# brendisurfs/Distributed-Backtesting-Exploration

Hardware: AMD Instinct MI355X
Metric: bar-evals/sec (symbols x params x bars) (higher is better)
Workload: dtype f64+int64; 1 GPU; BASELINE config 2: SMA fast/slow crossover, 5,000 symbols x 2,520 daily bars x 400 params per GPU; symbols_total=5000, symbols_per_gpu=5000, bars=2520, params=400, topk=100, parallelism=dp1 (contiguous symbol shards; exchange: none)

## Files before the change

distributed-backtesting-exploration_amd/csrc/analysis.cpp:

```cpp
#include <algorithm>
#include <cstring>
#include <string>
#include <vector>

#include "covariance.h"
#include "engine_state.h"
#include "portfolio.h"
#include "replay.h"
#include "surface.h"
#include "topk_rules.h"
#include "walkfwd.h"

using namespace bt;

namespace {

[[noreturn]] void refuse(const char* fn, const std::string& why) { throw HipFail{std::string(fn) + ": " + why}; }

uint8_t* enter(bt_engine* e, size_t staging_bytes) {
    activate(e);
    sync_all(e);
    e->d_arena.ensure(staging_bytes);
    return e->d_arena.p;
}

template <class F>
void for_chunks(size_t n, size_t per, F fn) {
    for (size_t i0 = 0; i0 < n; i0 += per) fn(i0, std::min(per, n - i0));
}

int32_t replay_impl(bt_engine* e, int32_t n, const bt_lane* lanes, int32_t trade_cap, bt_summary* sum,
                    int32_t* n_bars, bt_trade* trades, int64_t* equity, int8_t* pos, int64_t stride) {
    const char* fn = "bt_replay";
    if (!e) refuse(fn, "null engine");
    std::string why = replay_refusal(!e->syms.empty(), n, trade_cap, trades != nullptr, lanes != nullptr, sum != nullptr);
    if (!why.empty()) refuse(fn, why);
    if (n == 0) return 0;
    std::vector<ReplayLane> req;
    int32_t W = 0;
    why = replay_resolve(e->syms.data(), e->syms.size(), e->P, n, lanes, equity || pos, stride, req, W);
    if (!why.empty()) refuse(fn, why);
    const ReplayPlan pl = plan_replay(n, W, trade_cap, stride, equity != nullptr, pos != nullptr);
    uint8_t* base = enter(e, pl.staging_bytes);
    const size_t dcap = (size_t)pl.dcap, pitch = (size_t)pl.pitch;
    ReplayLane* d_lanes = at<ReplayLane>(base, pl.o_lane);
    ReplayOut out{};
    out.sum = at<bt_summary>(base, pl.o_sum);
    out.trades = dcap ? at<bt_trade>(base, pl.o_trades) : nullptr;
    out.trade_cap = (int32_t)dcap;
    out.equity = equity ? at<int64_t>(base, pl.o_equity) : nullptr;
    out.pos = pos ? at<int8_t>(base, pl.o_pos) : nullptr;
    out.pitch = pl.pitch;
    auto fetch = [&](void* dst, size_t dst_pitch, const void* src, size_t src_pitch, size_t m) {
        if (dst_pitch == src_pitch) {
            HIPCHK(hipMemcpyAsync(dst, src, m * src_pitch, hipMemcpyDeviceToHost, e->stream));
            return;
        }
        HIPCHK(hipMemcpy2DAsync(dst, dst_pitch, src, src_pitch, src_pitch, m, hipMemcpyDeviceToHost, e->stream));
        for (size_t i = 0; i < m; ++i)
            memset(static_cast<uint8_t*>(dst) + i * dst_pitch + src_pitch, 0, dst_pitch - src_pitch);
    };
    for_chunks((size_t)n, (size_t)pl.lanes_per_chunk, [&](size_t i0, size_t m) {
        HIPCHK(hipMemcpyAsync(d_lanes, req.data() + i0, m * sizeof(ReplayLane), hipMemcpyHostToDevice, e->stream));
        if (dcap) HIPCHK(hipMemsetAsync(out.trades, 0, m * dcap * sizeof(bt_trade), e->stream));
        if (equity) HIPCHK(hipMemsetAsync(out.equity, 0, m * pitch * 8, e->stream));
        if (pos) HIPCHK(hipMemsetAsync(out.pos, 0, m * pitch, e->stream));
        HIPCHK(launch_replay(d_lanes, (int32_t)m, e->d_h.p, e->d_l.p, e->d_c.p, e->grid, out, e->stream));
        HIPCHK(hipMemcpyAsync(sum + i0, out.sum, m * sizeof(bt_summary), hipMemcpyDeviceToHost, e->stream));
        if (dcap)
            fetch(trades + i0 * (size_t)trade_cap, (size_t)trade_cap * sizeof(bt_trade), out.trades,
                  dcap * sizeof(bt_trade), m);
        if (equity) fetch(equity + i0 * (size_t)stride, (size_t)stride * 8, out.equity, pitch * 8, m);
        if (pos) fetch(pos + i0 * (size_t)stride, (size_t)stride, out.pos, pitch, m);
        HIPCHK(hipStreamSynchronize(e->stream));
    });
    if (n_bars)
        for (int32_t i = 0; i < n; ++i) n_bars[i] = req[i].bars;
    return n;
}

void surface_launch(bt_engine* e, const SurfacePlan& pl, uint8_t* base, const bt_summary* d_sum,
                    const int32_t* d_ids, int32_t id_stride, int32_t S, int32_t P, bt_param_agg* agg,
                    bt_topk_rec* best) {
    SurfaceWork w{};
    w.partial = at<bt_param_agg>(base, pl.o_partial);
    w.fold = at<bt_param_agg>(base, pl.o_fold);
    w.best_partial = at<bt_topk_rec>(base, pl.o_best_partial);
    w.agg = agg ? at<bt_param_agg>(base, pl.o_agg) : nullptr;
    w.best = best ? at<bt_topk_rec>(base, pl.o_best) : nullptr;
    HIPCHK(launch_surface(d_sum, d_ids, id_stride, S, P, pl, w, e->stream));
    const size_t n_agg = (size_t)P * sizeof(bt_param_agg), n_best = (size_t)S * sizeof(bt_topk_rec);
    const size_t lo = agg ? pl.o_agg : pl.o_best, hi = best && S > 0 ? pl.o_best + n_best : pl.o_agg + n_agg;
    if (hi <= lo) return;
    e->h_surface.ensure(hi - lo);
    HIPCHK(hipMemcpyAsync(e->h_surface.p, base + lo, hi - lo, hipMemcpyDeviceToHost, e->stream));
    HIPCHK(hipStreamSynchronize(e->stream));
    if (agg) memcpy(agg, e->h_surface.p + (pl.o_agg - lo), n_agg);
    if (best && S > 0) memcpy(best, e->h_surface.p + (pl.o_best - lo), n_best);
}

int32_t surface_impl(bt_engine* e, bt_param_agg* agg, bt_topk_rec* best) {
    const char* fn = "bt_surface";
    if (!e) refuse(fn, "null engine");
    if (!e->ran) refuse(fn, "no results");
    uint64_t rows = 0;
    for (const SymDesc& sd : e->syms) rows += (uint64_t)sd.bars;
    const int32_t S = (int32_t)e->syms.size();
    const std::string why = surface_refusal(S, e->P, agg || best, false, rows);
    if (!why.empty()) refuse(fn, why);
    const SurfacePlan pl = plan_surface(S, e->P, e->cus, e->surface_chunks);
    uint8_t* base = enter(e, pl.staging_bytes);
    static_assert(sizeof(SymDesc) == 16 && offsetof(SymDesc, id) == 12, "SymDesc layout");
    surface_launch(e, pl, base, e->d_sum[e->cur].p, reinterpret_cast<const int32_t*>(e->d_syms.p) + 3, 4, S,
                   e->P, agg, best);
    return 0;
}

int32_t surface_of_impl(bt_engine* e, int32_t S, int32_t P, const bt_summary* sum, const int32_t* ids,
                        bt_param_agg* agg, bt_topk_rec* best) {
    const char* fn = "bt_surface_of";
    if (!e) refuse(fn, "null engine");
    const std::string why = surface_refusal(S, P, agg || best, true, 0);
    if (!why.empty()) refuse(fn, why);
    if (S > 0 && (!sum || !ids)) refuse(fn, "sum and sym_ids are required");
    const SurfacePlan pl = plan_surface(S, P, e->cus, e->surface_chunks, true);
    uint8_t* base = enter(e, pl.staging_bytes);
    bt_summary* d_sum = at<bt_summary>(base, pl.o_sum);
    int32_t* d_ids = at<int32_t>(base, pl.o_ids);
    if (S > 0) {
        HIPCHK(hipMemcpyAsync(d_sum, sum, (size_t)S * (size_t)P * sizeof(bt_summary), hipMemcpyHostToDevice, e->stream));
        HIPCHK(hipMemcpyAsync(d_ids, ids, (size_t)S * sizeof(int32_t), hipMemcpyHostToDevice, e->stream));
    }
    surface_launch(e, pl, base, d_sum, d_ids, 1, S, P, agg, best);
    return 0;
}

int32_t topk_of_impl(bt_engine* e, int32_t S, int32_t P, const bt_summary* sum, const int32_t* ids, int32_t k,
                     int32_t lds_free_hist, bt_topk_rec* out) {
    static_assert(kTopkOfMaxK == kTopkMax, "topk_rules.h restates kTopkMax");
    const char* fn = "bt_topk_of";
    if (!e) refuse(fn, "null engine");
    const std::string why = topk_of_refusal(S, P, k, sum != nullptr, ids, out != nullptr);
    if (!why.empty()) refuse(fn, why);
    const size_t n = (size_t)S * (size_t)P;
    std::vector<uint64_t> key(n);
    for (size_t i = 0; i < n; ++i) key[i] = order_key(sum[i].sharpe);
    std::vector<SymDesc> syms((size_t)S);
    for (int32_t s = 0; s < S; ++s) syms[s] = SymDesc{0, 0, ids[s]};
    const TopkOfPlan pl = plan_topk_of(S, P);
    uint8_t* base = enter(e, pl.staging_bytes);
    uint64_t* d_key = at<uint64_t>(base, pl.o_key);
    bt_summary* d_sum = at<bt_summary>(base, pl.o_sum);
    SymDesc* d_syms = at<SymDesc>(base, pl.o_syms);
    bt_topk_rec* d_out = at<bt_topk_rec>(base, pl.o_out);
    const TopkWork w{at<unsigned int>(base, pl.o_hist),      at<unsigned long long>(base, pl.o_state),
                     at<unsigned int>(base, pl.o_counts),    at<unsigned long long>(base, pl.o_above),
                     at<unsigned long long>(base, pl.o_cand), kTopkCap, d_out + 1, reinterpret_cast<int32_t*>(d_out)};
    HIPCHK(hipMemcpyAsync(d_key, key.data(), n * sizeof(uint64_t), hipMemcpyHostToDevice, e->stream));
    HIPCHK(hipMemcpyAsync(d_sum, sum, n * sizeof(bt_summary), hipMemcpyHostToDevice, e->stream));
    HIPCHK(hipMemcpyAsync(d_syms, syms.data(), (size_t)S * sizeof(SymDesc), hipMemcpyHostToDevice, e->stream));
    HIPCHK(hipMemsetAsync(d_out, 0, ((size_t)kTopkMax + 1) * sizeof(bt_topk_rec), e->stream));
    HIPCHK(launch_topk_init(w, e->stream));
    HIPCHK(launch_topk(d_key, d_sum, d_syms, (int64_t)n, P, k, w, e->stream, lds_free_hist != 0));
    std::vector<bt_topk_rec> got((size_t)k + 1);
    HIPCHK(hipMemcpyAsync(got.data(), d_out, got.size() * sizeof(bt_topk_rec), hipMemcpyDeviceToHost, e->stream));
    HIPCHK(hipStreamSynchronize(e->stream));
    int32_t count;
    memcpy(&count, &got[0], sizeof count);
    if (count < 0 || count > k) refuse(fn, "the device wrote a count of " + std::to_string(count));
    memcpy(out, got.data() + 1, (size_t)count * sizeof(bt_topk_rec));
    return count;
}

int32_t walk_forward_impl(bt_engine* e, int32_t K, const int32_t* bounds, int32_t train, bt_fold* folds,
                          bt_wf_step* steps, bt_fold* total) {
    const char* fn = "bt_walk_forward";
    if (!e) refuse(fn, "null engine");
    if (e->syms.empty()) refuse(fn, "no dataset loaded");
    if (K >= 1 && !bounds) refuse(fn, "bounds are required");
    const int32_t S = (int32_t)e->syms.size(), P = e->P;
    const std::string why = walkfwd_refusal(K, bounds, train, folds != nullptr, steps != nullptr,
                                            total != nullptr, S, P);
    if (!why.empty()) refuse(fn, why);
    const WalkfwdPlan pl = plan_walkfwd(S, P, K, e->max_bars, e->cus, e->walkfwd_budget);
    if (pl.rows_per_chunk < 1)
        refuse(fn, "P*K = " + std::to_string(P) + "*" + std::to_string(K) + " records of one row exceed the staging budget of " +
                       std::to_string(e->walkfwd_budget > 0 ? (size_t)e->walkfwd_budget : kWalkfwdBudget) + " bytes");
    uint8_t* base = enter(e, pl.staging_bytes);
    const bool select = steps || total;
    const int32_t n_steps = select ? walkfwd_steps(K, train) : 0;
    const size_t row_recs = (size_t)K * (size_t)P;
    HIPCHK(hipMemcpyAsync(base, bounds, ((size_t)K + 1) * sizeof(int32_t), hipMemcpyHostToDevice, e->stream));
    WfArgs a{};
    a.bounds = at<const int32_t>(base, 0);
    a.rec = at<bt_fold>(base, pl.o_rec);
    a.steps = at<bt_wf_step>(base, pl.o_steps);
    a.P = P, a.K = K;
    a.train = train, a.j0 = std::max(train, 1), a.n_steps = n_steps;
    std::vector<bt_fold> h_rec(folds ? (size_t)pl.rows_per_chunk * row_recs : 0);
    std::vector<bt_wf_step> own(!steps && total ? (size_t)S * (size_t)n_steps : 0);
    bt_wf_step* st = steps ? steps : own.data();
    for_chunks((size_t)S, (size_t)pl.rows_per_chunk, [&](size_t r0, size_t m) {
        a.syms = e->d_syms.p + r0;
        a.n_rows = (int32_t)m;
        HIPCHK(hipMemsetAsync(a.rec, 0, m * row_recs * sizeof(bt_fold), e->stream));
        HIPCHK(launch_wf_walk(a, e->d_h.p, e->d_l.p, e->d_c.p, e->grid, e->stream));
        if (select) {
            HIPCHK(launch_wf_select(a, e->grid, pl, e->stream));
            HIPCHK(hipMemcpyAsync(st + r0 * (size_t)n_steps, a.steps, m * (size_t)n_steps * sizeof(bt_wf_step),
                                  hipMemcpyDeviceToHost, e->stream));
        }
        if (folds)
            HIPCHK(hipMemcpyAsync(h_rec.data(), a.rec, m * row_recs * sizeof(bt_fold), hipMemcpyDeviceToHost, e->stream));
        HIPCHK(hipStreamSynchronize(e->stream));
        if (folds)
            for (size_t r = 0; r < m; ++r)
                for (size_t k = 0; k < (size_t)K; ++k)
                    for (size_t p = 0; p < (size_t)P; ++p)
                        folds[((r0 + r) * (size_t)P + p) * (size_t)K + k] = h_rec[(r * (size_t)K + k) * (size_t)P + p];
    });
    if (total) walkfwd_totals(S, n_steps, st, e->grid.sqrt_ann, total);
    return 0;
}

int32_t portfolio_impl(bt_engine* e, int32_t n, const bt_pf_lane* lanes, int32_t T, int64_t* pnl, int64_t* equity,
                       int32_t* n_long, int32_t* n_short, bt_pf_summary* summary) {
    const char* fn = "bt_portfolio";
    if (!e) refuse(fn, "null engine");
    std::string why = portfolio_refusal(!e->syms.empty(), n, lanes != nullptr, T,
                                        pnl || equity || n_long || n_short || summary);
    if (!why.empty()) refuse(fn, why);
    PfResolved rs;
    why = portfolio_resolve(e->syms.data(), e->syms.size(), e->P, n, lanes, T, rs);
    if (!why.empty()) refuse(fn, why);
    const int32_t m = (int32_t)rs.req.size();
    const PortfolioPlan pl = plan_portfolio(m, T, e->cus, e->portfolio_replicas);
    uint8_t* base = enter(e, pl.staging_bytes);
    e->h_portfolio.ensure(pl.out_bytes);
    PfLane* d_lanes = at<PfLane>(base, pl.o_lanes);
    PfWork w{};
    w.acc_pnl = at<unsigned long long>(base, pl.o_acc_pnl);
    w.acc_cnt = at<unsigned long long>(base, pl.o_acc_cnt);
    w.pitch = pl.pitch;
    w.R = pl.R;
    w.T = T;
    w.n_lanes = rs.n_lanes, w.lo = rs.lo, w.hi = rs.hi;
    w.pnl = at<int64_t>(base, pl.o_pnl);
    w.equity = at<int64_t>(base, pl.o_equity);
    w.n_long = at<int32_t>(base, pl.o_long);
    w.n_short = at<int32_t>(base, pl.o_short);
    w.sum = at<bt_pf_summary>(base, pl.o_sum);
    if (m > 0)
        HIPCHK(hipMemcpyAsync(d_lanes, rs.req.data(), (size_t)m * sizeof(PfLane), hipMemcpyHostToDevice, e->stream));
    HIPCHK(hipMemsetAsync(base + pl.o_acc_pnl, 0, pl.acc_bytes, e->stream));
    HIPCHK(launch_portfolio(d_lanes, m, e->d_h.p, e->d_l.p, e->d_c.p, e->grid, w, pl, e->stream));
    HIPCHK(hipMemcpyAsync(e->h_portfolio.p, base + pl.o_pnl, pl.out_bytes, hipMemcpyDeviceToHost, e->stream));
    HIPCHK(hipStreamSynchronize(e->stream));
    const uint8_t* h = e->h_portfolio.p;
    const size_t bars = (size_t)T;
    if (pnl) memcpy(pnl, h, bars * 8);
    if (equity) memcpy(equity, h + (pl.o_equity - pl.o_pnl), bars * 8);
    if (n_long) memcpy(n_long, h + (pl.o_long - pl.o_pnl), bars * 4);
    if (n_short) memcpy(n_short, h + (pl.o_short - pl.o_pnl), bars * 4);
    if (summary) memcpy(summary, h + (pl.o_sum - pl.o_pnl), sizeof *summary);
    return 0;
}

GramWork gram_work(uint8_t* base, const GramPlan& pl, int32_t n, int32_t T) {
    GramWork w{};
    w.D = at<int32_t>(base, pl.o_d);
    w.pitch = pl.pitch;
    w.partial = at<bt_wide>(base, pl.o_partial);
    w.gram = at<bt_wide>(base, pl.o_gram);
    w.sums = at<int64_t>(base, pl.o_sums);
    w.n = n, w.T = T;
    w.nt = pl.nt, w.tiles = pl.tiles;
    w.chunks = pl.chunks, w.chunk_bars = pl.chunk_bars;
    return w;
}

void gram_fetch(bt_engine* e, uint8_t* base, const GramPlan& pl, int32_t n, bt_wide* gram, int64_t* sums) {
    e->h_gram.ensure(pl.out_bytes);
    HIPCHK(hipMemcpyAsync(e->h_gram.p, base + pl.o_gram, pl.out_bytes, hipMemcpyDeviceToHost, e->stream));
    HIPCHK(hipStreamSynchronize(e->stream));
    if (gram) memcpy(gram, e->h_gram.p, (size_t)n * (size_t)n * sizeof(bt_wide));
    if (sums) memcpy(sums, e->h_gram.p + (pl.o_sums - pl.o_gram), (size_t)n * sizeof(int64_t));
}

int32_t covariance_impl(bt_engine* e, int32_t n, const bt_lane* lanes, int32_t from_bar, int32_t to_bar,
                        bt_wide* gram, int64_t* sums, int32_t* T_out) {
    const char* fn = "bt_covariance";
    if (!e) refuse(fn, "null engine");
    std::string why = covariance_refusal(!e->syms.empty(), n, lanes != nullptr, from_bar, to_bar, gram || sums || T_out);
    if (!why.empty()) refuse(fn, why);
    std::vector<ReplayLane> req;
    int32_t W = 0, T = 0;
    why = replay_resolve(e->syms.data(), e->syms.size(), e->P, n, lanes, false, 0, req, W);
    if (!why.empty()) refuse(fn, why);
    why = covariance_window(from_bar, to_bar, W, T);
    if (!why.empty()) refuse(fn, why);
    const GramPlan pl = plan_gram(n, T, e->cus, e->gram_split);
    why = gram_staging_refusal(pl.staging_bytes, kGramStagingMax, n, T);
    if (!why.empty()) refuse(fn, why);
    if (T_out) *T_out = T;
    if (n == 0 || T == 0) {
        if (gram) memset(gram, 0, (size_t)n * (size_t)n * sizeof(bt_wide));
        if (sums) memset(sums, 0, (size_t)n * sizeof(int64_t));
        return 0;
    }
    uint8_t* base = enter(e, pl.staging_bytes);
    ReplayLane* d_lanes = at<ReplayLane>(base, pl.o_lanes);
    const GramWork w = gram_work(base, pl, n, T);
    HIPCHK(hipMemcpyAsync(d_lanes, req.data(), (size_t)n * sizeof(ReplayLane), hipMemcpyHostToDevice, e->stream));
    HIPCHK(hipMemsetAsync(base + pl.o_d, 0, pl.d_bytes, e->stream));
    HIPCHK(launch_gram_walk(d_lanes, e->d_h.p, e->d_l.p, e->d_c.p, e->grid, w, from_bar, from_bar + T, e->stream));
    HIPCHK(launch_gram(w, pl, false, e->stream));
    gram_fetch(e, base, pl, n, gram, sums);
    return 0;
}

int32_t gram_of_impl(bt_engine* e, int32_t n, int32_t T, const int32_t* d, bt_wide* gram, int64_t* sums) {
    const char* fn = "bt_gram_of";
    if (!e) refuse(fn, "null engine");
    std::string why = gram_of_refusal(n, T, d != nullptr, gram || sums);
    if (!why.empty()) refuse(fn, why);
    const GramPlan pl = plan_gram(n, T, e->cus, e->gram_split);
    why = gram_staging_refusal(pl.staging_bytes, kGramStagingMax, n, T);
    if (!why.empty()) refuse(fn, why);
    if (n == 0 || T == 0) {
        if (gram) memset(gram, 0, (size_t)n * (size_t)n * sizeof(bt_wide));
        if (sums) memset(sums, 0, (size_t)n * sizeof(int64_t));
        return 0;
    }
    why = gram_domain_refusal(n, T, d);
    if (!why.empty()) refuse(fn, why);
    uint8_t* base = enter(e, pl.staging_bytes);
    const GramWork w = gram_work(base, pl, n, T);
    HIPCHK(hipMemsetAsync(base + pl.o_d, 0, pl.d_bytes, e->stream));
    HIPCHK(hipMemcpy2DAsync(w.D, (size_t)pl.pitch * sizeof(int32_t), d, (size_t)T * sizeof(int32_t),
                            (size_t)T * sizeof(int32_t), (size_t)n, hipMemcpyHostToDevice, e->stream));
    HIPCHK(launch_gram(w, pl, true, e->stream));
    gram_fetch(e, base, pl, n, gram, sums);
    return 0;
}

}

extern "C" {

int32_t bt_covariance(bt_engine* e, int32_t n, const bt_lane* lanes, int32_t from_bar, int32_t to_bar, bt_wide* gram,
                      int64_t* sums, int32_t* T_out) {
    ABI_GUARD(-1, { return covariance_impl(e, n, lanes, from_bar, to_bar, gram, sums, T_out); })
}

int32_t bt_gram_of(bt_engine* e, int32_t n, int32_t T, const int32_t* d, bt_wide* gram, int64_t* sums) {
    ABI_GUARD(-1, { return gram_of_impl(e, n, T, d, gram, sums); })
}

int32_t bt_set_gram_split(bt_engine* e, int32_t k) {
    ABI_GUARD(-1, {
        if (!e) refuse("bt_set_gram_split", "null engine");
        if (k < 0) refuse("bt_set_gram_split", "k = " + std::to_string(k) + " is negative");
        e->gram_split = k;
        return 0;
    })
}

int32_t bt_portfolio(bt_engine* e, int32_t n, const bt_pf_lane* lanes, int32_t T, int64_t* pnl, int64_t* equity,
                     int32_t* n_long, int32_t* n_short, bt_pf_summary* summary) {
    ABI_GUARD(-1, { return portfolio_impl(e, n, lanes, T, pnl, equity, n_long, n_short, summary); })
}

int32_t bt_set_portfolio_replicas(bt_engine* e, int32_t r) {
    ABI_GUARD(-1, {
        if (!e) refuse("bt_set_portfolio_replicas", "null engine");
        if (r < 0) refuse("bt_set_portfolio_replicas", "r = " + std::to_string(r) + " is negative");
        e->portfolio_replicas = r;
        return 0;
    })
}

int32_t bt_replay(bt_engine* e, int32_t n, const bt_lane* lanes, int32_t trade_cap, bt_summary* sum,
                  int32_t* n_bars, bt_trade* trades, int64_t* equity, int8_t* pos, int64_t stride) {
    ABI_GUARD(-1, { return replay_impl(e, n, lanes, trade_cap, sum, n_bars, trades, equity, pos, stride); })
}

int32_t bt_surface(bt_engine* e, bt_param_agg* agg, bt_topk_rec* best) {
    ABI_GUARD(-1, { return surface_impl(e, agg, best); })
}

int32_t bt_surface_of(bt_engine* e, int32_t S, int32_t P, const bt_summary* sum, const int32_t* sym_ids,
                      bt_param_agg* agg, bt_topk_rec* best) {
    ABI_GUARD(-1, { return surface_of_impl(e, S, P, sum, sym_ids, agg, best); })
}

int32_t bt_topk_of(bt_engine* e, int32_t S, int32_t P, const bt_summary* sum, const int32_t* sym_ids, int32_t k,
                   int32_t lds_free_hist, bt_topk_rec* out) {
    ABI_GUARD(-1, { return topk_of_impl(e, S, P, sum, sym_ids, k, lds_free_hist, out); })
}

int32_t bt_walk_forward(bt_engine* e, int32_t K, const int32_t* bounds, int32_t train, bt_fold* folds,
                        bt_wf_step* steps, bt_fold* total) {
    ABI_GUARD(-1, { return walk_forward_impl(e, K, bounds, train, folds, steps, total); })
}

int32_t bt_set_walkfwd_budget(bt_engine* e, int64_t bytes) {
    ABI_GUARD(-1, {
        if (!e) refuse("bt_set_walkfwd_budget", "null engine");
        if (bytes < 0) refuse("bt_set_walkfwd_budget", "bytes = " + std::to_string(bytes) + " is negative");
        e->walkfwd_budget = bytes;
        return 0;
    })
}

int32_t bt_set_surface_chunks(bt_engine* e, int32_t chunks) {
    ABI_GUARD(-1, {
        if (!e) refuse("bt_set_surface_chunks", "null engine");
        if (chunks < 0) refuse("bt_set_surface_chunks", "chunks = " + std::to_string(chunks) + " is negative");
        e->surface_chunks = chunks;
        return 0;
    })
}

}
```

distributed-backtesting-exploration_amd/csrc/engine.cpp:

```cpp
#include <algorithm>
#include <cmath>
#include <cstdio>
#include <cstdlib>
#include <cstring>
#include <memory>
#include <string>
#include <vector>

#include "batch.h"
#include "csv.h"
#include "engine_state.h"
#include "topk_rules.h"

using namespace bt;

static thread_local std::string g_err;

void bt::set_last_error(const std::string& s) { g_err = s; }

namespace {

const char* kernel_name(int32_t strategy) {
    switch (strategy) {
        case BT_SMA_CROSS: return "bt::sma_kernel";
        case BT_EMA_OLS: return "bt::ema_tile_kernel";
        default: return "bt::boll_tile_kernel";
    }
}

std::string validate_and_copy(bt_engine* e, const bt_config& c) {
    const std::string err = plan_grid(c, e->grid);
    if (!err.empty()) return err;
    AxisSpec ax[4];
    const int nax = config_axes(c, ax);
    for (int i = 0; i < nax; ++i) e->ax[i].assign(ax[i].v, ax[i].v + ax[i].n);
    e->P = e->grid.n_params;
    if (c.annualization <= 0) return "annualization must be positive";
    e->grid.sqrt_ann = std::sqrt((double)c.annualization);
    if (c.topk < 0 || c.topk > kTopkMax) return "topk must be in [0, 1024]";
    if ((c.flags & BT_FLAG_PARITY) && c.trade_cap <= 0) return "parity mode needs trade_cap > 0";
    return "";
}

void upload_grid(bt_engine* e) {
    const int32_t** dst[4] = {&e->grid.a, &e->grid.b, &e->grid.c, &e->grid.d};
    for (int i = 0; i < 4; ++i) {
        *dst[i] = nullptr;
        if (e->ax[i].empty()) continue;
        e->d_axes[i].ensure(e->ax[i].size());
        HIPCHK(hipMemcpy(e->d_axes[i].p, e->ax[i].data(), e->ax[i].size() * 4, hipMemcpyHostToDevice));
        *dst[i] = e->d_axes[i].p;
    }
    e->grid.kwin = nullptr;
    e->grid.krecip = nullptr;
    if (e->cfg.strategy == BT_SMA_CROSS) {
        std::vector<int32_t> win(e->ax[0]);
        win.insert(win.end(), e->ax[1].begin(), e->ax[1].end());
        win.resize((win.size() + kKeyGrab - 1) / kKeyGrab * kKeyGrab, 1);
        std::vector<double> recip(win.size());
        for (size_t i = 0; i < win.size(); ++i) recip[i] = key_recip(win[i]);
        e->d_kwin.ensure(win.size());
        e->d_krecip.ensure(win.size());
        HIPCHK(hipMemcpy(e->d_kwin.p, win.data(), win.size() * sizeof(int32_t), hipMemcpyHostToDevice));
        HIPCHK(hipMemcpy(e->d_krecip.p, recip.data(), recip.size() * sizeof(double), hipMemcpyHostToDevice));
        e->grid.kwin = e->d_kwin.p;
        e->grid.krecip = e->d_krecip.p;
    }
}

static_assert(kStageAlign == kRowAlign, "batch.h lays staging rows out as the device columns");

void set_dataset(bt_engine* e, std::vector<SymDesc>&& syms, int64_t rows) {
    sync_all(e);
    e->syms = std::move(syms);
    e->rows = rows;
    e->max_bars = 0;
    for (const SymDesc& sd : e->syms) e->max_bars = std::max(e->max_bars, sd.bars);
    const size_t n_sym = e->syms.size();
    e->d_syms.ensure(std::max<size_t>(1, n_sym));
    if (n_sym)
        HIPCHK(hipMemcpyAsync(e->d_syms.p, e->syms.data(), n_sym * sizeof(SymDesc),
                              hipMemcpyHostToDevice, e->stream));
    const size_t r = std::max<int64_t>(1, rows);
    e->d_c.ensure(r);
    if (has_hl(e)) {
        e->d_h.ensure(r);
        e->d_l.ensure(r);
    }
    e->ran = false;
}

void layout(bt_engine* e, int32_t n_sym, const int32_t* bars, const int64_t* ids) {
    std::vector<SymDesc> syms((size_t)n_sym);
    int64_t off = 0;
    for (int32_t s = 0; s < n_sym; ++s) {
        syms[s].off = off;
        syms[s].bars = bars[s];
        syms[s].id = (int32_t)ids[s];
        off += align_rows(bars[s]);
    }
    set_dataset(e, std::move(syms), off);
}

TopkWork topk_work(bt_engine* e) {
    return TopkWork{e->d_hist.p, e->d_state.p, e->d_counts.p, e->d_above.p, e->d_cand.p,
                    kTopkCap, e->d_top.p + 1, reinterpret_cast<int32_t*>(e->d_top.p)};
}

void ensure_outputs(bt_engine* e) {
    const size_t n = (size_t)e->syms.size() * e->P;
    for (int b = 0; b < 2; ++b) {
        e->d_sum[b].ensure(std::max<size_t>(1, n));
        e->d_key[b].ensure(std::max<size_t>(1, n));
    }
    e->d_ntr_ring.ensure(kNtrRing);
    if (e->cfg.flags & BT_FLAG_PARITY) {
        e->d_sums.ensure(std::max<size_t>(1, n));
        e->d_trades.ensure(std::max<size_t>(1, n * (size_t)e->cfg.trade_cap));
    }
    if (e->cfg.topk > 0 && !e->topk_ready) {
        e->d_hist.ensure(4096);
        e->d_counts.ensure(2);
        e->d_state.ensure(4);
        e->d_above.ensure(kTopkCap);
        e->d_cand.ensure(kTopkCap);
        e->d_top.ensure(kTopkMax + 1);
        e->h_top.ensure(kTopkMax + 1);
        HIPCHK(launch_topk_init(topk_work(e), e->stream));
        e->topk_ready = true;
    }
}

void run_impl(bt_engine* e) {
    activate(e);
    ensure_outputs(e);
    const int32_t S = (int32_t)e->syms.size();
    const int64_t run = e->nrun++;
    const int b = (int)(run & 1);
    e->cur = b;
    if (e->tdone_armed[b] && hipEventQuery(e->ev_tdone[b]) != hipSuccess)
        HIPCHK(hipStreamWaitEvent(e->stream, e->ev_tdone[b], 0));
    Out out{};
    out.sum = e->d_sum[b].p;
    out.key = e->d_key[b].p;
    const bool parity = (e->cfg.flags & BT_FLAG_PARITY) != 0;
    out.sums = parity ? e->d_sums.p : nullptr;
    out.trades = parity ? e->d_trades.p : nullptr;
    out.trade_cap = parity ? e->cfg.trade_cap : 0;
    const int slot = (int)(run % kNtrRing);
    if (slot % (kNtrRing / 2) == 0)
        HIPCHK(hipMemsetAsync(e->d_ntr_ring.p + slot, 0, (kNtrRing / 2) * sizeof(unsigned long long),
                              e->stream));
    e->ntr[b] = e->d_ntr_ring.p + slot;
    out.n_trades = e->ntr[b];
    out.dbg = nullptr;
    if (BT_ABL(e->grid, 64)) {
        e->d_dbg.ensure(kDbgSlots + 8 * kDbgBlocks);
        HIPCHK(hipMemsetAsync(e->d_dbg.p, 0, (kDbgSlots + 8 * kDbgBlocks) * sizeof(unsigned long long),
                              e->stream));
        out.dbg = e->d_dbg.p;
    }
    const bool timing = (e->cfg.flags & BT_FLAG_TIMING) != 0;
    std::pair<Event, Event> ev;
    if (timing) {
        if (!e->ev_pool.empty()) {
            ev = std::move(e->ev_pool.back());
            e->ev_pool.pop_back();
        }
        ev.first.ensure(0);
        ev.second.ensure(0);
        HIPCHK(hipEventRecord(ev.first, e->stream));
    }
    const LaunchPlan pl = plan_launch(e->grid, e->ax[0].data(),
                                      RunShape{S, e->max_bars, parity, e->seg_req, e->burn_req, e->cus});
    SegArgs sg{nullptr, nullptr, nullptr, nullptr, pl.G, pl.burn_tiles};
    if (pl.G > 1) {
        e->d_seg.ensure(pl.seg_slots);
        sg.rec = e->d_seg.p;
        if (pl.pos_bytes) sg.pos = reinterpret_cast<int8_t*>(e->d_seg.p) + pl.pos_off;
        if (pl.ema_doubles) {
            e->d_segema.ensure(pl.ema_doubles);
            sg.ema = e->d_segema.p;
        }
        e->d_refixed.ensure(1);
        HIPCHK(hipMemsetAsync(e->d_refixed.p, 0, sizeof(unsigned long long), e->stream));
        sg.refixed = e->d_refixed.p;
    }
    e->seg_last = pl.G;
    hipError_t err;
    switch (e->cfg.strategy) {
        case BT_SMA_CROSS:
            err = launch_sma(e->d_syms.p, S, e->d_c.p, e->grid, out, parity, sg, pl, e->stream);
            break;
        case BT_EMA_OLS:
            err = launch_ema_ols(e->d_syms.p, S, e->d_c.p, e->grid, out, parity, sg, pl, e->stream);
            break;
        default:
            err = launch_boll(e->d_syms.p, S, e->d_h.p, e->d_l.p, e->d_c.p, e->grid, out, parity, sg, pl,
                              e->stream);
            break;
    }
    HIPCHK(err);
    hipEvent_t kdone = e->ev_kdone;
    if (timing) {
        HIPCHK(hipEventRecord(ev.second, e->stream));
        kdone = ev.second;
        e->ev_pending.push_back(std::move(ev));
    }
    if (e->cfg.topk > 0) {
        if (!timing) HIPCHK(hipEventRecord(kdone, e->stream));
        HIPCHK(hipStreamWaitEvent(e->tstream, kdone, 0));
        HIPCHK(launch_topk(e->d_key[b].p, e->d_sum[b].p, e->d_syms.p, (int64_t)S * e->P, e->P,
                           e->cfg.topk, topk_work(e), e->tstream, pl.topk_lds_free));
        HIPCHK(hipEventRecord(e->ev_tdone[b], e->tstream));
        e->tdone_armed[b] = true;
    }
    e->ran = true;
}

void drain_timing(bt_engine* e) {
    for (auto& ev : e->ev_pending) {
        HIPCHK(hipEventSynchronize(ev.second));
        float ms = 0.f;
        HIPCHK(hipEventElapsedTime(&ms, ev.first, ev.second));
        e->kernel_ms += ms;
        e->launches += 1;
        e->ev_pool.push_back(std::move(ev));
    }
    e->ev_pending.clear();
}


std::vector<bt_topk_rec> read_topk_impl(bt_engine* e, int32_t k) {
    if (!e->ran || e->cfg.topk <= 0) throw HipFail{"top-k not computed (topk == 0 or no run)"};
    const size_t nrec = (size_t)e->cfg.topk + 1;
    HIPCHK(hipMemcpyAsync(e->h_top.p, e->d_top.p, nrec * sizeof(bt_topk_rec), hipMemcpyDeviceToHost,
                          e->tstream));
    sync_all(e);
    int32_t n = 0;
    memcpy(&n, e->h_top.p, sizeof n);
    if (n < 0 || n > e->cfg.topk) throw HipFail{"device top-k returned a bad record count"};
    std::vector<bt_topk_rec> res(e->h_top.p + 1, e->h_top.p + 1 + n);
    if ((int32_t)res.size() > k) res.resize(k);
    return res;
}

void run_batch_impl(bt_engine* e, size_t n, const bt_job_in* jobs, bt_job_out* outs) {
    Batch bat(n, jobs, e->cfg.host_threads);
    activate(e);
    sync_all(e);
    const int64_t rows = bat.parse();
    const int ncol = has_hl(e) ? 3 : 1;
    for (int k = 0; k < ncol; ++k) e->h_stage[k].ensure((size_t)rows);
    bat.stage(e->h_stage[0].p, ncol == 3 ? e->h_stage[1].p : nullptr, ncol == 3 ? e->h_stage[2].p : nullptr);
    bt_batch_profile& pr = bat.prof;
    e->n_errors = pr.n_failed;
    const size_t nres = bat.syms.size() * (size_t)e->P;
    if (!bat.syms.empty()) {
        std::vector<SymDesc> syms;
        for (const StagedSym& s : bat.syms) syms.push_back(SymDesc{s.row, s.bars, (int32_t)syms.size()});
        for (Event& ev : e->ev_batch) ev.ensure(0);
        e->h_sum.ensure(nres);
        set_dataset(e, std::move(syms), rows);
        HIPCHK(hipEventRecord(e->ev_batch[0], e->stream));
        int32_t* dst[3] = {e->d_c.p, e->d_h.p, e->d_l.p};
        for (int k = 0; k < ncol; ++k)
            HIPCHK(hipMemcpyAsync(dst[k], e->h_stage[k].p, (size_t)rows * 4, hipMemcpyHostToDevice,
                                  e->stream));
        HIPCHK(hipEventRecord(e->ev_batch[1], e->stream));
        run_impl(e);
        HIPCHK(hipEventRecord(e->ev_batch[2], e->stream));
        HIPCHK(hipMemcpyAsync(e->h_sum.p, e->d_sum[e->cur].p, nres * sizeof(bt_summary),
                              hipMemcpyDeviceToHost, e->stream));
        HIPCHK(hipEventRecord(e->ev_batch[3], e->stream));
        sync_all(e);
        float ms = 0.f;
        HIPCHK(hipEventElapsedTime(&ms, e->ev_batch[0], e->ev_batch[1]));
        pr.upload_ms = ms;
        HIPCHK(hipEventElapsedTime(&ms, e->ev_batch[1], e->ev_batch[2]));
        pr.compute_ms = ms;
        HIPCHK(hipEventElapsedTime(&ms, e->ev_batch[2], e->ev_batch[3]));
        pr.readback_ms = ms;
    }
    bat.format(e->h_sum.p, e->P, outs);
    e->prof = pr;
}

}

bool bt::engine_exchange_view(bt_engine* e, ExchangeView& v, std::string& err) {
    if (!e || !e->ran || e->cfg.topk <= 0 || !e->d_top.p) {
        err = "exchange needs an engine with topk > 0 and a finished bt_run";
        return false;
    }
    v.tstream = e->tstream;
    v.device = e->cfg.device;
    v.topk = e->cfg.topk;
    v.d_top = e->d_top.p;
    v.d_ntr = e->ntr[e->cur];
    v.bar_evals = 0;
    for (const SymDesc& s : e->syms) v.bar_evals += (int64_t)s.bars * e->P;
    return true;
}

void bt::engine_exchange_enqueued(bt_engine* e) {
    if (hipEventRecord(e->ev_tdone[e->cur], e->tstream) == hipSuccess) e->tdone_armed[e->cur] = true;
}

extern "C" {

int32_t bt_abi_version(void) { return BT_ABI_VERSION; }

const char* bt_last_error(void) { return g_err.c_str(); }

static bt_engine* create_impl(const bt_config* cfg) {
    if (cfg == nullptr) throw HipFail{"null config"};
    auto e = std::make_unique<bt_engine>();
    e->cfg = *cfg;
    const std::string m = validate_and_copy(e.get(), *cfg);
    if (!m.empty()) throw HipFail{m};
    e->cfg.fast = e->cfg.slow = e->cfg.span = e->cfg.ols = nullptr;
    e->cfg.bwin = e->cfg.k_num = e->cfg.sl_bps = e->cfg.tp_bps = nullptr;
    int ndev = 0;
    HIPCHK(hipGetDeviceCount(&ndev));
    if (cfg->device < 0 || cfg->device >= ndev)
        throw HipFail{"HIP device " + std::to_string(cfg->device) + " not present (" +
                      std::to_string(ndev) + " visible)"};
    activate(e.get());
    if (hipDeviceGetAttribute(&e->cus, hipDeviceAttributeMultiprocessorCount, cfg->device) != hipSuccess ||
        e->cus <= 0)
        e->cus = kCusFallback;
    if (cfg->stream)
        e->stream.borrow((hipStream_t)cfg->stream);
    else
        e->stream.create();
    e->tstream.create();
    e->ev_kdone.ensure(hipEventDisableTiming);
    for (Event& ev : e->ev_tdone) ev.ensure(hipEventDisableTiming);
    upload_grid(e.get());
#ifdef BT_PROFILING
    if (const char* ab = getenv("BT_ABLATE")) e->grid.ablate = atoi(ab);
#endif
    return e.release();
}

bt_engine* bt_engine_create(const bt_config* cfg, char* err, size_t errlen) {
    auto failed = [&]() -> bt_engine* {
        if (err && errlen) snprintf(err, errlen, "%s", g_err.c_str());
        return nullptr;
    };
    ABI_GUARD(failed(), { return create_impl(cfg); })
}

void bt_engine_destroy(bt_engine* e) {
    if (!e) return;
    try {
        delete e;
    } catch (...) {
    }
}

int32_t bt_num_params(const bt_engine* e) { return e ? e->P : -1; }

int32_t bt_set_segments(bt_engine* e, int32_t segments, int32_t burn_tiles) {
    ABI_GUARD(-1, {
        if (!e || segments < 0 || segments > 64 || burn_tiles < 0) throw HipFail{"bad arguments"};
        e->seg_req = segments;
        e->burn_req = burn_tiles;
        return 0;
    })
}

int32_t bt_last_segments(bt_engine* e, int64_t* refixed_blocks) {
    ABI_GUARD(-1, {
        if (!e) throw HipFail{"null engine"};
        if (refixed_blocks) {
            unsigned long long n = 0;
            if (e->seg_last > 1 && e->d_refixed.p) {
                activate(e);
                sync_all(e);
                HIPCHK(hipMemcpy(&n, e->d_refixed.p, sizeof n, hipMemcpyDeviceToHost));
            }
            *refixed_blocks = (int64_t)n;
        }
        return e->seg_last;
    })
}

int32_t bt_load_synthetic(bt_engine* e, uint64_t seed, int64_t sym_begin, int32_t n_sym,
                          int32_t n_bars, int32_t freq) {
    ABI_GUARD(-1, {
        if (!e) throw HipFail{"null engine"};
        if (n_sym < 0 || n_bars < 1 || n_bars > kMaxBars) throw HipFail{"bad synthetic shape"};
        if (sym_begin < 0 || sym_begin + n_sym > (1LL << 31)) throw HipFail{"bad symbol ids"};
        if (freq != BT_DAILY && freq != BT_MINUTE) throw HipFail{"bad freq"};
        activate(e);
        std::vector<int32_t> bars(n_sym, n_bars);
        std::vector<int64_t> ids(n_sym);
        for (int32_t s = 0; s < n_sym; ++s) ids[s] = sym_begin + s;
        layout(e, n_sym, bars.data(), ids.data());
        HIPCHK(launch_gen(e->d_syms.p, n_sym, seed, freq, nullptr, has_hl(e) ? e->d_h.p : nullptr,
                          has_hl(e) ? e->d_l.p : nullptr, e->d_c.p, e->stream));
        sync_all(e);
        return 0;
    })
}

int32_t bt_load_ohlc(bt_engine* e, int32_t n_sym, const int64_t* sym_ids, const int32_t* bars,
                     const int64_t* row_off, const int32_t* h, const int32_t* l, const int32_t* c) {
    ABI_GUARD(-1, {
        if (!e || n_sym < 0 || (n_sym > 0 && (!sym_ids || !bars || !row_off || !c)))
            throw HipFail{"bad arguments"};
        if (has_hl(e) && (!h || !l)) throw HipFail{"strategy needs high and low columns"};
        for (int32_t s = 0; s < n_sym; ++s)
            if (bars[s] < 1 || bars[s] > kMaxBars) throw HipFail{"bad bar count"};
        const std::string bad_id = sym_id_refusal(n_sym, sym_ids);
        if (!bad_id.empty()) throw HipFail{"bt_load_ohlc: " + bad_id};
        activate(e);
        sync_all(e);
        layout(e, n_sym, bars, sym_ids);
        const int ncol = has_hl(e) ? 3 : 1;
        const int32_t* src[3] = {c, h, l};
        int32_t* dst[3] = {e->d_c.p, e->d_h.p, e->d_l.p};
        if (e->rows > 0) {
            for (int k = 0; k < ncol; ++k) {
                e->h_stage[k].ensure((size_t)e->rows);
                for (int32_t s = 0; s < n_sym; ++s)
                    memcpy(e->h_stage[k].p + e->syms[s].off, src[k] + row_off[s], (size_t)bars[s] * 4);
                HIPCHK(hipMemcpyAsync(dst[k], e->h_stage[k].p, (size_t)e->rows * 4,
                                      hipMemcpyHostToDevice, e->stream));
            }
            sync_all(e);
        }
        return 0;
    })
}

int32_t bt_run(bt_engine* e) {
    ABI_GUARD(-1, {
        if (!e) throw HipFail{"null engine"};
        run_impl(e);
        return 0;
    })
}

int32_t bt_sync(bt_engine* e) {
    ABI_GUARD(-1, {
        if (!e) throw HipFail{"null engine"};
        activate(e);
        sync_all(e);
        return 0;
    })
}

int32_t bt_read_summaries(bt_engine* e, bt_summary* out, size_t n) {
    ABI_GUARD(-1, {
        if (!e || !e->ran) throw HipFail{"no results"};
        const size_t have = e->syms.size() * (size_t)e->P;
        if (n > have) throw HipFail{"n exceeds symbols x params"};
        activate(e);
        sync_all(e);
        HIPCHK(hipMemcpy(out, e->d_sum[e->cur].p, n * sizeof(bt_summary), hipMemcpyDeviceToHost));
        return 0;
    })
}

int32_t bt_read_sums(bt_engine* e, bt_sums* out, size_t n) {
    ABI_GUARD(-1, {
        if (!e || !e->ran || !(e->cfg.flags & BT_FLAG_PARITY)) throw HipFail{"no parity results"};
        if (n > e->syms.size() * (size_t)e->P) throw HipFail{"n too large"};
        activate(e);
        sync_all(e);
        HIPCHK(hipMemcpy(out, e->d_sums.p, n * sizeof(bt_sums), hipMemcpyDeviceToHost));
        return 0;
    })
}

int32_t bt_read_trades(bt_engine* e, bt_trade* out, size_t n) {
    ABI_GUARD(-1, {
        if (!e || !e->ran || !(e->cfg.flags & BT_FLAG_PARITY)) throw HipFail{"no parity results"};
        if (n > e->syms.size() * (size_t)e->P * e->cfg.trade_cap) throw HipFail{"n too large"};
        activate(e);
        sync_all(e);
        HIPCHK(hipMemcpy(out, e->d_trades.p, n * sizeof(bt_trade), hipMemcpyDeviceToHost));
        return 0;
    })
}

int32_t bt_read_topk(bt_engine* e, bt_topk_rec* out, int32_t k) {
    ABI_GUARD(-1, {
        if (!e || !out || k <= 0) throw HipFail{"bad arguments"};
        activate(e);
        std::vector<bt_topk_rec> r = read_topk_impl(e, std::min(k, e->cfg.topk));
        std::copy(r.begin(), r.end(), out);
        return (int32_t)r.size();
    })
}

int32_t bt_topk_fetch_async(bt_engine* e, int32_t slot) {
    ABI_GUARD(-1, {
        if (!e || slot < 0 || slot >= BT_PIPE_SLOTS) throw HipFail{"bad arguments"};
        if (!e->ran || e->cfg.topk <= 0) throw HipFail{"top-k not computed (topk == 0 or no run)"};
        activate(e);
        e->h_slot[slot].ensure(kTopkMax + 2);
        e->slot_ev[slot].ensure(hipEventDisableTiming);
        bt_topk_rec* h = e->h_slot[slot].p;
        HIPCHK(hipMemcpyAsync(h, e->d_top.p, ((size_t)e->cfg.topk + 1) * sizeof(bt_topk_rec),
                              hipMemcpyDeviceToHost, e->tstream));
        HIPCHK(hipMemcpyAsync(h + kTopkMax + 1, e->ntr[e->cur], sizeof(unsigned long long),
                              hipMemcpyDeviceToHost, e->tstream));
        HIPCHK(hipEventRecord(e->slot_ev[slot], e->tstream));
        HIPCHK(hipEventRecord(e->ev_tdone[e->cur], e->tstream));
        e->slot_armed[slot] = true;
        return 0;
    })
}

int32_t bt_topk_fetch_wait(bt_engine* e, int32_t slot, bt_topk_rec* out, int32_t k,
                           int64_t* n_trades) {
    ABI_GUARD(-1, {
        if (!e || slot < 0 || slot >= BT_PIPE_SLOTS || !out || k <= 0) throw HipFail{"bad arguments"};
        if (!e->slot_armed[slot]) throw HipFail{"no fetch pending on this slot"};
        activate(e);
        HIPCHK(hipEventSynchronize(e->slot_ev[slot]));
        const bt_topk_rec* h = e->h_slot[slot].p;
        int32_t n = 0;
        memcpy(&n, h, sizeof n);
        if (n < 0 || n > e->cfg.topk) throw HipFail{"device top-k returned a bad record count"};
        const int32_t m = std::min(n, std::min(k, e->cfg.topk));
        std::copy(h + 1, h + 1 + m, out);
        if (n_trades) {
            unsigned long long t = 0;
            memcpy(&t, h + kTopkMax + 1, sizeof t);
            *n_trades = (int64_t)t;
        }
        return m;
    })
}

int32_t bt_read_stats(bt_engine* e, bt_stats* out) {
    ABI_GUARD(-1, {
        if (!e || !out) throw HipFail{"bad arguments"};
        activate(e);
        sync_all(e);
        bt_stats st{};
        st.n_symbols = (int64_t)e->syms.size();
        st.n_params = e->P;
        for (const SymDesc& s : e->syms) st.bar_evals += (int64_t)s.bars * e->P;
        st.errors = e->n_errors;
        if (e->ran) {
            unsigned long long n = 0;
            HIPCHK(hipMemcpy(&n, e->ntr[e->cur], sizeof n, hipMemcpyDeviceToHost));
            st.trades = (int64_t)n;
        }
        *out = st;
        return 0;
    })
}

int32_t bt_read_close(bt_engine* e, int32_t sym_index, int32_t* out, int32_t n) {
    ABI_GUARD(-1, {
        if (!e || sym_index < 0 || sym_index >= (int32_t)e->syms.size()) throw HipFail{"bad symbol"};
        const SymDesc& sd = e->syms[sym_index];
        if (n > sd.bars) throw HipFail{"n exceeds bars"};
        activate(e);
        sync_all(e);
        HIPCHK(hipMemcpy(out, e->d_c.p + sd.off, (size_t)n * 4, hipMemcpyDeviceToHost));
        return 0;
    })
}

int32_t bt_read_debug(bt_engine* e, uint64_t* out, int32_t n) {
    ABI_GUARD(-1, {
        if (!e || !out || n < 0 || n > kDbgSlots + 8 * kDbgBlocks || !e->d_dbg.p) throw HipFail{"no debug stamps"};
        activate(e);
        sync_all(e);
        HIPCHK(hipMemcpy(out, e->d_dbg.p, (size_t)n * 8, hipMemcpyDeviceToHost));
        return 0;
    })
}

int32_t bt_kernel_timing(bt_engine* e, double* total_ms, int64_t* launches, const char** name) {
    ABI_GUARD(-1, {
        if (!e) throw HipFail{"null engine"};
        activate(e);
        drain_timing(e);
        if (total_ms) *total_ms = e->kernel_ms;
        if (launches) *launches = e->launches;
        if (name) *name = kernel_name(e->cfg.strategy);
        return 0;
    })
}

int32_t bt_reset_timing(bt_engine* e) {
    ABI_GUARD(-1, {
        if (!e) throw HipFail{"null engine"};
        activate(e);
        drain_timing(e);
        e->kernel_ms = 0.0;
        e->launches = 0;
        return 0;
    })
}

int32_t bt_run_batch(bt_engine* e, size_t n, const bt_job_in* jobs, bt_job_out* outs) {
    ABI_GUARD(-1, {
        if (!e || (n > 0 && (!jobs || !outs))) throw HipFail{"bad arguments"};
        for (size_t i = 0; i < n; ++i) outs[i] = bt_job_out{nullptr, 0, 0, 0};
        try {
            run_batch_impl(e, n, jobs, outs);
        } catch (...) {
            bt_job_out_free(outs, n);
            throw;
        }
        return 0;
    })
}

int32_t bt_last_batch_profile(bt_engine* e, bt_batch_profile* out) {
    ABI_GUARD(-1, {
        if (!e || !out) throw HipFail{"bad arguments"};
        *out = e->prof;
        return 0;
    })
}

int64_t bt_format_summaries(const bt_summary* r, int32_t P, char* out, size_t cap) {
    ABI_GUARD(-1, {
        if (P < 0) throw HipFail{"bad arguments"};
        if (!out) return (int64_t)((size_t)P * kLineMax);
        if (P > 0 && !r) throw HipFail{"bad arguments"};
        if (cap < (size_t)P * kLineMax) throw HipFail{"output buffer too small"};
        return (int64_t)fmt_job_into(r, P, out);
    })
}

void bt_job_out_free(bt_job_out* outs, size_t n) {
    if (outs) free_job_outs(outs, n);
}

int32_t bt_merge_topk(const bt_topk_rec* in, size_t n, int32_t k, bt_topk_rec* out) {
    ABI_GUARD(-1, {
        if ((n > 0 && !in) || !out || k < 0) throw HipFail{"bad arguments"};
        std::vector<bt_topk_rec> v(in, in + n);
        std::sort(v.begin(), v.end(), topk_less);
        const size_t m = std::min<size_t>(v.size(), (size_t)k);
        std::copy(v.begin(), v.begin() + m, out);
        return (int32_t)m;
    })
}

double bt_i128_to_double(uint64_t lo, int64_t hi) { return i128_to_double(lo, hi); }

int32_t bt_parse_csv(const uint8_t* buf, size_t len, int32_t cap, int32_t* h, int32_t* l,
                     int32_t* c, char* err, size_t errlen) {
    return bt_parse_job(buf, len, cap, h, l, c, err, errlen);
}

int64_t bt_encode_columns(const int32_t* o, const int32_t* h, const int32_t* l, const int32_t* c,
                          const int64_t* v, int32_t n, uint8_t* out, size_t cap) {
    ABI_GUARD(-1, {
        if (n < 1 || n > kMaxBars || !o || !h || !l || !c) throw HipFail{"bad arguments"};
        const size_t need = binary_payload_size(n, v != nullptr);
        if (!out) return (int64_t)need;
        if (cap < need) throw HipFail{"output buffer too small"};
        return (int64_t)encode_binary(o, h, l, c, v, n, out);
    })
}

int64_t bt_gen_payload(uint64_t seed, int64_t sym, int32_t bars, int32_t freq, uint8_t* out,
                       size_t cap) {
    ABI_GUARD(-1, {
        if (bars < 1 || bars > kMaxBars || (freq != BT_DAILY && freq != BT_MINUTE))
            throw HipFail{"bad arguments"};
        const size_t need = binary_payload_size(bars, true);
        if (!out) return (int64_t)need;
        if (cap < need) throw HipFail{"output buffer too small"};
        std::vector<int32_t> o((size_t)bars), h((size_t)bars), l((size_t)bars), c((size_t)bars);
        std::vector<int64_t> v((size_t)bars);
        gen_host(seed, sym, bars, freq, o.data(), h.data(), l.data(), c.data(), v.data());
        return (int64_t)encode_binary(o.data(), h.data(), l.data(), c.data(), v.data(), bars, out);
    })
}

int32_t bt_parse_job(const uint8_t* buf, size_t len, int32_t cap, int32_t* h, int32_t* l,
                     int32_t* c, char* err, size_t errlen) {
    ABI_GUARD(-1, {
        Bars b;
        std::string m;
        if (!parse_job(buf, len, b, m)) {
            if (err && errlen) snprintf(err, errlen, "%s", m.c_str());
            set_last_error(m);
            return -1;
        }
        if ((int64_t)b.c.size() > cap) throw HipFail{"cap too small"};
        if (h) memcpy(h, b.h.data(), b.h.size() * 4);
        if (l) memcpy(l, b.l.data(), b.l.size() * 4);
        if (c) memcpy(c, b.c.data(), b.c.size() * 4);
        return (int32_t)b.c.size();
    })
}

}
```

distributed-backtesting-exploration_amd/csrc/engine_state.h:

```cpp
#pragma once
#include <hip/hip_runtime.h>

#include <utility>
#include <vector>

#include "hip_owned.h"
#include "internal.h"
#include "plan.h"

namespace bt {

constexpr int64_t kNtrRing = 64;

struct EngineState {
    bt_config cfg{};
    std::vector<int32_t> ax[4];
    Grid grid{};
    int32_t P = 0;
    Stream tstream, stream;
    ~EngineState() {
        if (!stream) return;
        (void)hipSetDevice(cfg.device);
        (void)hipStreamSynchronize(stream);
        if (tstream) (void)hipStreamSynchronize(tstream);
    }
    DevBuf<int32_t> d_axes[4];
    DevBuf<int32_t> d_kwin;
    DevBuf<double> d_krecip;
    std::vector<SymDesc> syms;
    int64_t rows = 0;
    DevBuf<SymDesc> d_syms;
    DevBuf<int32_t> d_c, d_h, d_l;
    DevBuf<bt_summary> d_sum[2];
    DevBuf<uint64_t> d_key[2];
    DevBuf<unsigned long long> d_ntr_ring;
    unsigned long long* ntr[2] = {nullptr, nullptr};
    int cur = 0;
    int64_t nrun = 0;
    DevBuf<bt_sums> d_sums;
    DevBuf<bt_trade> d_trades;
    int cus = kCusFallback;
    int32_t max_bars = 0;
    int32_t seg_req = 0, burn_req = 0, seg_last = 1;
    DevBuf<SegRec> d_seg;
    DevBuf<double> d_segema;
    DevBuf<unsigned long long> d_refixed;
    DevBuf<unsigned long long> d_dbg;
    Event ev_kdone;
    Event ev_tdone[2];
    bool tdone_armed[2] = {false, false};
    DevBuf<unsigned int> d_hist, d_counts;
    DevBuf<unsigned long long> d_state, d_above, d_cand;
    DevBuf<bt_topk_rec> d_top;
    PinnedBuf<bt_topk_rec> h_top;
    PinnedBuf<bt_topk_rec> h_slot[BT_PIPE_SLOTS];
    Event slot_ev[BT_PIPE_SLOTS];
    bool slot_armed[BT_PIPE_SLOTS] = {};
    bool topk_ready = false;
    bool ran = false;
    std::vector<std::pair<Event, Event>> ev_pending, ev_pool;
    double kernel_ms = 0.0;
    int64_t launches = 0;
    PinnedBuf<int32_t> h_stage[3];
    PinnedBuf<bt_summary> h_sum;
    Event ev_batch[4];
    bt_batch_profile prof{};
    int64_t n_errors = 0;
    DevBuf<uint8_t> d_arena;
    int32_t surface_chunks = 0;
    PinnedBuf<uint8_t> h_surface;
    int64_t walkfwd_budget = 0;
    int32_t portfolio_replicas = 0;
    PinnedBuf<uint8_t> h_portfolio;
    int32_t gram_split = 0;
    PinnedBuf<uint8_t> h_gram;
};

}

struct bt_engine : bt::EngineState {};

namespace bt {

inline void activate(bt_engine* e) { HIPCHK(hipSetDevice(e->cfg.device)); }

inline bool has_hl(const bt_engine* e) { return e->cfg.strategy == BT_BOLL; }

inline void sync_all(bt_engine* e) {
    HIPCHK(hipStreamSynchronize(e->stream));
    if (e->tstream) HIPCHK(hipStreamSynchronize(e->tstream));
}

template <class T>
T* at(uint8_t* base, size_t off) { return reinterpret_cast<T*>(base + off); }

}
```

distributed-backtesting-exploration_amd/csrc/plan.cpp:

```cpp
#include "plan.h"

#include <algorithm>
#include <cmath>
#include <cstdlib>

#include "batch.h"
#include "csv.h"
#include "lds_layout.h"

namespace bt {

namespace {

constexpr int kDefaultBurnTiles = 64;
constexpr int kSmaBurnTiles = 2;

uint32_t next_pow2(uint32_t x) {
    uint32_t r = 1;
    while (r < x) r <<= 1;
    return r;
}

size_t ema_lds_bytes(const Grid& g, int ts) { return tile_lds_layout(0, g.ring, g.na, g.nb, 0, ts).total; }

}

int config_axes(const bt_config& c, AxisSpec ax[4]) {
    switch (c.strategy) {
        case BT_SMA_CROSS:
            ax[0] = {c.fast, c.n_fast, "fast", 1, kMaxBars};
            ax[1] = {c.slow, c.n_slow, "slow", 1, kMaxBars};
            return 2;
        case BT_EMA_OLS:
            ax[0] = {c.span, c.n_span, "span", 1, kMaxBars};
            ax[1] = {c.ols, c.n_ols, "ols", 1, 1 << 16};
            return 2;
        case BT_BOLL:
            ax[0] = {c.bwin, c.n_bwin, "bwin", 1, 1 << 16};
            ax[1] = {c.k_num, c.n_k, "k_num", 0, 1 << 20};
            ax[2] = {c.sl_bps, c.n_sl, "sl_bps", 0, 9999};
            ax[3] = {c.tp_bps, c.n_tp, "tp_bps", 0, 9999};
            return 4;
        default:
            return 0;
    }
}

std::string plan_grid(const bt_config& c, Grid& g) {
    AxisSpec ax[4];
    const int nax = config_axes(c, ax);
    if (nax == 0) return "unknown strategy";
    for (int i = 0; i < nax; ++i) {
        if (ax[i].n <= 0 || ax[i].v == nullptr) return std::string("empty axis: ") + ax[i].what;
        for (int32_t j = 0; j < ax[i].n; ++j)
            if (ax[i].v[j] < ax[i].lo || ax[i].v[j] > ax[i].hi)
                return std::string("value out of range on axis ") + ax[i].what + ": " + std::to_string(ax[i].v[j]);
    }
    auto amax = [&](int i) { return *std::max_element(ax[i].v, ax[i].v + ax[i].n); };
    g.strategy = c.strategy;
    g.na = ax[0].n;
    g.nb = ax[1].n;
    g.nc = nax > 2 ? ax[2].n : 1;
    g.nd = nax > 3 ? ax[3].n : 1;
    switch (c.strategy) {
        case BT_SMA_CROSS:
            g.wmax = std::max(amax(0), amax(1));
            g.ring = (int32_t)next_pow2((uint32_t)g.wmax + 3 * kTile);
            if (sma_lds_layout(g.ring, g.na + g.nb).total > kCuLdsBytes)
                return "SMA grid needs more LDS than a CU has (windows too long)";
            break;
        case BT_EMA_OLS:
            if (c.band_bps < 0 || c.band_bps >= 10000) return "band_bps out of range";
            if (c.n_span > 64) return "EMA grid: at most 64 spans (one helper lane per span)";
            g.band_bps = c.band_bps;
            g.wmax = amax(1);
            g.ring = (g.wmax + 5 * kTile - 1) / kTile * kTile;
            if (ema_lds_bytes(g, 1) > kCuLdsBytes) return "EMA grid needs more LDS than a CU has (OLS windows too long)";
            break;
        default: {
            if (c.k_den < 1 || c.k_den > (1 << 20)) return "k_den out of range";
            g.k_den = c.k_den;
            g.wmax = amax(0);
            const int64_t kmax = std::max<int64_t>(c.k_den, amax(1));
            if ((int64_t)g.wmax * kmax >= (1LL << 32)) return "Bollinger grid outside the exact int128 range (window * k >= 2^32)";
            g.ring = (g.wmax + 4 * kTile - 1) / kTile * kTile;
            for (int q = 0; q < 8; ++q) {
                const int64_t kn = q < c.n_k ? c.k_num[q] : 0;
                g.kn2[q] = (double)(kn * kn);
            }
            g.kmin_idx = (int32_t)(std::min_element(c.k_num, c.k_num + c.n_k) - c.k_num);
            if (tile_lds_layout(1, g.ring, g.na, g.nb, g.nc + g.nd).total > kCuLdsBytes)
                return "Bollinger grid needs more LDS than a CU has (windows too long)";
            break;
        }
    }
    const int64_t P = (int64_t)g.na * g.nb * g.nc * g.nd;
    if (P <= 0 || P > (1 << 20)) return "parameter grid too large";
    g.n_params = (int32_t)P;
    return "";
}

namespace {

size_t seg_records(const LaunchPlan& pl, const Grid& g, const RunShape& r) {
    return pl.G > 1 ? (size_t)pl.G * r.n_sym * g.n_params : 0;
}

struct SmaShape {
    int pw;
    int dedicated;
    int block, gy;
};

SmaShape sma_shape(int P) {
    const int need = (P + 63) / 64;
    SmaShape s;
    if (need == 16) {
        s.pw = 16;
        s.dedicated = 0;
    } else {
        const int nby = (need + 14) / 15;
        s.pw = (need + nby - 1) / nby;
        s.dedicated = 1;
    }
    s.block = 64 * (s.pw + s.dedicated);
    s.gy = (P + 64 * s.pw - 1) / (64 * s.pw);
    return s;
}

int32_t sma_auto_segments(int32_t n_sym, const SmaShape& sh, int32_t max_bars, int32_t wmax,
                          int32_t burn_tiles, int cus) {
    if (n_sym <= 0) return 1;
    if (sh.block <= 512) return 1;
    constexpr double kSegRounds = 28.0;
    const double rounds = (double)n_sym * sh.gy / cus;
    if (rounds >= kSegRounds) return 1;
    int G = std::min(8, (int)std::ceil(kSegRounds / rounds));
    const int ntiles = (max_bars + kTile - 1) / kTile;
    const int lookback = (wmax - 1 + kTile - 1) / kTile;
    while (G > 1 && burn_tiles + 0.05 * lookback > 0.02 * ntiles / G) --G;
    return G;
}

void plan_sma(const Grid& g, const RunShape& r, LaunchPlan& pl) {
    const SmaShape sh = sma_shape(g.n_params);
    pl.burn_tiles = r.burn_req > 0 ? r.burn_req : kSmaBurnTiles;
    if (!r.parity)
        pl.G = r.seg_req > 0 ? r.seg_req
                             : sma_auto_segments(r.n_sym, sh, r.max_bars, g.wmax, pl.burn_tiles, r.cus);
    pl.grid_y = sh.gy;
    pl.block = sh.block;
    pl.dedicated = sh.dedicated;
    pl.lds = sma_lds_layout(g.ring, g.na + g.nb).total;
    pl.one_trip = sh.block > 512;
#ifdef BT_PROFILING
    if (BT_ABL(g, 128)) pl.lds = std::max(pl.lds, (size_t)(g.ablate & 256 ? 80 : 60) * 1024);
    if (const char* v = getenv("BT_ONE_TRIP")) pl.one_trip = atoi(v) != 0;
#endif
    const size_t nrec = seg_records(pl, g, r);
    pl.pos_off = nrec * sizeof(SegRec);
    pl.pos_bytes = 2 * nrec;
    pl.seg_slots = nrec + (pl.pos_bytes + sizeof(SegRec) - 1) / sizeof(SegRec);
}

int tile_param_waves(int need, int cap) {
    int pw = std::min(need, cap);
#ifdef BT_PROFILING
    if (const char* v = getenv("BT_PW")) pw = std::max(1, std::min(atoi(v), pw));
#endif
    return pw;
}

int tile_extra_waves(int used, int x) {
#ifdef BT_PROFILING
    if (const char* v = getenv("BT_XW")) x = atoi(v);
#endif
    return std::max(0, std::min(x, 16 - used));
}

int tile_lanes_per_wave() {
    int l = 64;
#ifdef BT_PROFILING
    if (const char* v = getenv("BT_LPW")) l = std::max(1, std::min(atoi(v), 64));
#endif
    return l;
}

uint32_t boll_wave_map(int pw, int nsplit, int xw) {
    uint32_t m = 0;
    for (int w = 0; w < 8; ++w) m |= (uint32_t)w << (4 * w);
    const int nw = pw + 1 + nsplit + xw;
    if (nw == 8 && pw == 4) {
        const int split_map[8] = {0, 1, 2, 3, 6, 7, 5, 4};
        const int plain_map[8] = {0, 1, 2, 3, 5, 6, 7, 4};
        const int* r = nsplit == 1 ? split_map : plain_map;
        m = 0;
        for (int w = 0; w < 8; ++w) m |= (uint32_t)r[w] << (4 * w);
    }
#ifdef BT_PROFILING
    if (const char* v = getenv("BT_WAVEMAP")) m = (uint32_t)strtoul(v, nullptr, 16);
#endif
    return m;
}

bool tile_split_walk() {
    bool on = true;
#ifdef BT_PROFILING
    if (const char* v = getenv("BT_SPLIT")) on = atoi(v) != 0;
#endif
    return on;
}

int32_t tile_auto_segments(int32_t n_sym, int32_t n_params, int32_t max_bars, int helpers,
                           int32_t burn_tiles, int cus) {
    if (n_sym <= 0) return 1;
    const int pw = std::min((n_params + 63) / 64, 1024 / 64 - helpers);
    const long long blocks = (long long)n_sym * ((n_params + 64 * pw - 1) / (64 * pw));
    if (blocks > cus) return 1;
    int G = (int)std::min<long long>(4, std::max<long long>(1, 2LL * cus / blocks));
    const int ntiles = (max_bars + kTile - 1) / kTile;
    while (G > 1 && ntiles / G < 2 * burn_tiles) --G;
    return G;
}

int32_t ema_burn_tiles(int32_t max_span) {
    return std::max(kDefaultBurnTiles, (6 * max_span + kTile - 1) / kTile);
}

int ema_stage_tiles(const Grid& g) {
    const size_t cu = kCuLdsBytes, l1 = ema_lds_bytes(g, 1), l2 = ema_lds_bytes(g, 2);
    return l2 <= cu && cu / l2 >= cu / l1 ? 2 : 1;
}

void plan_ema(const Grid& g, const int32_t* spans, const RunShape& r, LaunchPlan& pl) {
    int32_t maxspan = 1;
    for (int32_t i = 0; i < g.na; ++i) maxspan = std::max(maxspan, spans[i]);
    pl.burn_tiles = r.burn_req > 0 ? r.burn_req : ema_burn_tiles(maxspan);
    if (!r.parity)
        pl.G = r.seg_req > 0 ? r.seg_req
                             : tile_auto_segments(r.n_sym, g.n_params, r.max_bars, 2, pl.burn_tiles, r.cus);
    pl.lpw = tile_lanes_per_wave();
    const int pw = tile_param_waves((g.n_params + pl.lpw - 1) / pl.lpw, 1024 / 64 - 2);
    pl.xw = tile_extra_waves(pw + 2, 5);
    pl.grid_y = (g.n_params + pl.lpw * pw - 1) / (pl.lpw * pw);
    pl.block = 64 * (pw + 2 + pl.xw);
    pl.ts = ema_stage_tiles(g);
    pl.lds = ema_lds_bytes(g, pl.ts);
    pl.seg_slots = seg_records(pl, g, r);
    pl.ema_doubles = pl.G > 1 ? (size_t)pl.G * r.n_sym * kEmaSegStride : 0;
    pl.topk_lds_free = pl.ts == 2;
}

void plan_boll(const Grid& g, const RunShape& r, LaunchPlan& pl) {
    pl.burn_tiles = r.burn_req > 0 ? r.burn_req : kDefaultBurnTiles;
    if (!r.parity)
        pl.G = r.seg_req > 0 ? r.seg_req
                             : tile_auto_segments(r.n_sym, g.n_params, r.max_bars, 1, kDefaultBurnTiles, r.cus);
    pl.lpw = tile_lanes_per_wave();
    const int pw = tile_param_waves((g.n_params + pl.lpw - 1) / pl.lpw, 1024 / 64 - 1);
    pl.grid_y = (g.n_params + pl.lpw * pw - 1) / (pl.lpw * pw);
    if (tile_split_walk() && pw >= 2 && pl.grid_y == 1) {
        const long long per_k = (long long)g.na * g.nc * g.nd;
        const int grp = (int)((g.kmin_idx * per_k) / pl.lpw);
        if (grp < pw) pl.split_grp = grp;
    }
    const int nsplit = pl.split_grp < 0 ? 0 : 1;
    const int base = pw + 1 + nsplit;
    const bool sparse = (long long)r.n_sym * pl.grid_y * pl.G <= r.cus;
    pl.xw = tile_extra_waves(base, sparse ? 4 : std::max(2, std::min(3, 8 - base)));
    pl.block = 64 * (base + pl.xw);
    pl.lds = tile_lds_layout(1, g.ring, g.na, g.nb, g.nc + g.nd).total;
    pl.wmap = boll_wave_map(pw, nsplit, pl.xw);
    pl.seg_slots = seg_records(pl, g, r);
}

}

LaunchPlan plan_launch(const Grid& g, const int32_t* ax0, const RunShape& r) {
    LaunchPlan pl{};
    pl.G = 1;
    pl.split_grp = -1;
    switch (g.strategy) {
        case BT_SMA_CROSS: plan_sma(g, r, pl); break;
        case BT_EMA_OLS: plan_ema(g, ax0, r, pl); break;
        default: plan_boll(g, r, pl); break;
    }
    return pl;
}

SurfacePlan plan_surface(int32_t S, int32_t P, int cus, int32_t chunks_req, bool staged) {
    constexpr int kSurfaceWaves = 4, kSurfaceMinRows = 16;
    constexpr int32_t kMaxGridY = 65535;
    SurfacePlan pl{};
    S = std::max(S, 0);
    P = std::max(P, 1);
    pl.p_tiles = (P + 63) / 64;
    pl.block = 64 * std::min(pl.p_tiles, 4);
    pl.p_blocks = (P + pl.block - 1) / pl.block;
    int64_t chunks = chunks_req;
    if (chunks <= 0) {
        const int64_t waves_per_chunk = (int64_t)pl.p_blocks * (pl.block / 64);
        const int64_t want = ((int64_t)std::max(cus, 1) * 4 * kSurfaceWaves + waves_per_chunk - 1) / waves_per_chunk;
        chunks = std::min<int64_t>(want, S / kSurfaceMinRows);
    }
    chunks = std::max<int64_t>(1, std::min<int64_t>(chunks, std::min<int64_t>(S, kMaxGridY)));
    pl.chunks = (int32_t)chunks;
    pl.rows_per_chunk = S / pl.chunks;
    pl.rows_rem = S % pl.chunks;
    constexpr int kFoldDirect = 16;
    if (pl.chunks > kFoldDirect) pl.fold_ways = (int32_t)std::ceil(std::sqrt((double)pl.chunks));
    pl.partial_bytes = (size_t)pl.chunks * (size_t)P * sizeof(bt_param_agg);
    pl.fold_bytes = (size_t)pl.fold_ways * (size_t)P * sizeof(bt_param_agg);
    pl.best_partial_bytes = (size_t)S * (size_t)pl.p_tiles * sizeof(bt_topk_rec);
    Carve c;
    pl.o_partial = c.take(pl.partial_bytes);
    pl.o_fold = c.take(pl.fold_bytes);
    pl.o_best_partial = c.take(pl.best_partial_bytes);
    pl.o_agg = c.take((size_t)P * sizeof(bt_param_agg));
    pl.o_best = c.take((size_t)S * sizeof(bt_topk_rec));
    pl.o_sum = c.take(staged ? (size_t)S * (size_t)P * sizeof(bt_summary) : 0);
    pl.o_ids = c.take(staged ? (size_t)S * sizeof(int32_t) : 0);
    pl.staging_bytes = c.staging_bytes();
    return pl;
}

ReplayPlan plan_replay(int32_t n, int32_t W, int32_t trade_cap, int64_t stride, bool equity, bool pos,
                       size_t budget_req) {
    ReplayPlan pl{};
    n = std::max(n, 0);
    const size_t budget = budget_req > 0 ? budget_req : kReplayBudget;
    pl.dcap = std::max<int64_t>(0, std::min<int64_t>(trade_cap, W));
    pl.pitch = equity || pos ? std::min<int64_t>(stride, align_rows(W)) : 0;
    const size_t per_lane = sizeof(ReplayLane) + sizeof(bt_summary) + (size_t)pl.dcap * sizeof(bt_trade) +
                            (equity ? (size_t)pl.pitch * 8 : 0) + (pos ? (size_t)pl.pitch : 0);
    const size_t pad = 5 * kStagingAlign;
    const size_t lanes = std::min<size_t>((size_t)n, std::max<size_t>(1, budget > pad ? (budget - pad) / per_lane : 0));
    pl.lanes_per_chunk = (int32_t)lanes;
    pl.chunks = lanes ? (int32_t)(((size_t)n + lanes - 1) / lanes) : 0;
    Carve c;
    pl.o_lane = c.take(lanes * sizeof(ReplayLane));
    pl.o_sum = c.take(lanes * sizeof(bt_summary));
    pl.o_trades = c.take(lanes * (size_t)pl.dcap * sizeof(bt_trade));
    pl.o_equity = c.take(equity ? lanes * (size_t)pl.pitch * 8 : 0);
    pl.o_pos = c.take(pos ? lanes * (size_t)pl.pitch : 0);
    pl.staging_bytes = c.staging_bytes();
    return pl;
}

WalkfwdPlan plan_walkfwd(int32_t S, int32_t P, int32_t K, int32_t max_bars, int cus, int64_t budget_req) {
    constexpr int64_t kMaxGrid = 1LL << 30;
    WalkfwdPlan pl{};
    S = std::max(S, 0);
    P = std::max(P, 1);
    K = std::max(K, 1);
    const size_t budget = budget_req > 0 ? (size_t)budget_req : kWalkfwdBudget;
    Carve c;
    c.take(((size_t)K + 1) * sizeof(int32_t));
    pl.bounds_bytes = c.end;
    const size_t rec_bytes = (size_t)K * (size_t)P * sizeof(bt_fold), step_bytes = (size_t)(K - 1) * sizeof(bt_wf_step);
    pl.row_bytes = rec_bytes + step_bytes;
    const size_t fixed = pl.bounds_bytes + 2 * kStagingAlign;
    int64_t rows = budget > fixed ? (int64_t)((budget - fixed) / pl.row_bytes) : 0;
    rows = std::min<int64_t>(rows, kMaxGrid / std::max(P, K));
    rows = std::min<int64_t>(rows, S);
    pl.rows_per_chunk = (int32_t)rows;
    pl.chunks = rows > 0 ? (int32_t)((S + rows - 1) / rows) : 0;
    pl.sel_block = 64 * std::min((P + 63) / 64, 4);
    pl.tiles = (std::max(max_bars, 0) + kTile - 1) / kTile;
    pl.waves = rows * P;
    pl.fill = (double)pl.waves / ((double)std::max(cus, 1) * 4 * 8);
    pl.staging_bytes = rows > 0 ? fixed + (size_t)rows * pl.row_bytes : 0;
    pl.o_rec = c.take((size_t)rows * rec_bytes);
    pl.o_steps = c.take((size_t)rows * step_bytes);
    return pl;
}

PortfolioPlan plan_portfolio(int32_t n, int32_t T, int cus, int32_t replicas_req, size_t budget_req) {
    PortfolioPlan pl{};
    n = std::max(n, 0);
    T = std::max(T, 1);
    const size_t budget = budget_req > 0 ? budget_req : kPortfolioAccBudget;
    pl.tiles = (T + kTile - 1) / kTile;
    pl.pitch = (int64_t)pl.tiles * kTile;
    const size_t row = (size_t)pl.pitch * 16;
    int32_t R = 1;
    if (replicas_req > 0) {
        R = std::min(replicas_req, kPortfolioMaxReplicas);
        while (R > 1 && (size_t)R * row > budget) R /= 2;
    } else {
        while (R * 2 <= kPortfolioMaxReplicas && R * 2 <= n && (size_t)(R * 2) * row <= budget) R *= 2;
    }
    pl.R = R;
    pl.finish_block = (int32_t)std::min<int64_t>(pl.pitch, 1024);
    pl.fill = (double)n / ((double)std::max(cus, 1) * 4 * 8);
    Carve c;
    pl.o_lanes = c.take((size_t)n * sizeof(PfLane));
    pl.o_acc_pnl = c.take((size_t)R * (size_t)pl.pitch * 8);
    pl.o_acc_cnt = c.take((size_t)R * (size_t)pl.pitch * 8);
    pl.acc_bytes = c.end - pl.o_acc_pnl;
    pl.o_pnl = c.take((size_t)T * 8);
    pl.o_equity = c.take((size_t)T * 8);
    pl.o_long = c.take((size_t)T * 4);
    pl.o_short = c.take((size_t)T * 4);
    pl.o_sum = c.take(sizeof(bt_pf_summary));
    pl.out_bytes = pl.o_sum + sizeof(bt_pf_summary) - pl.o_pnl;
    pl.staging_bytes = c.staging_bytes();
    return pl;
}

GramPlan plan_gram(int32_t n, int32_t T, int cus, int32_t split_req) {
    GramPlan pl{};
    n = std::max(n, 0);
    T = std::max(T, 0);
    pl.nt = (n + 15) / 16;
    pl.tiles = pl.nt * (pl.nt + 1) / 2;
    const int64_t groups = std::max<int64_t>(1, ((int64_t)T + kTile - 1) / kTile);
    pl.pitch = groups * kTile;
    const size_t chunk_partial = (size_t)pl.tiles * 256 * sizeof(bt_wide);
    int64_t most = chunk_partial ? std::max<size_t>(1, kGramPartialBudget / chunk_partial) : 1;
    most = std::min<int64_t>(std::min<int64_t>(most, groups), 65535);
    int64_t chunks = 1;
    if (split_req > 0) {
        chunks = split_req;
    } else if (pl.tiles > 0) {
        const int64_t want = (int64_t)std::max(cus, 1) * kGramWavesPerCu;
        chunks = std::min<int64_t>((want + pl.tiles - 1) / pl.tiles, pl.pitch / kGramMinChunkBars);
    }
    chunks = std::max<int64_t>(1, std::min(chunks, most));
    const int64_t per = (groups + chunks - 1) / chunks;
    pl.chunk_bars = (int32_t)(per * kTile);
    pl.chunks = (int32_t)((groups + per - 1) / per);
    pl.fold_block = 256;
    pl.fill = (double)pl.tiles * pl.chunks / ((double)std::max(cus, 1) * kGramWavesPerCu);
    Carve c;
    pl.o_lanes = c.take((size_t)n * sizeof(ReplayLane));
    pl.o_d = c.take((size_t)n * (size_t)pl.pitch * sizeof(int32_t));
    pl.d_bytes = c.end - pl.o_d;
    pl.o_partial = c.take((size_t)pl.chunks * chunk_partial);
    pl.o_gram = c.take((size_t)n * (size_t)n * sizeof(bt_wide));
    pl.o_sums = c.take((size_t)n * sizeof(int64_t));
    pl.out_bytes = pl.o_sums + (size_t)n * sizeof(int64_t) - pl.o_gram;
    pl.staging_bytes = c.staging_bytes();
    return pl;
}

TopkOfPlan plan_topk_of(int32_t S, int32_t P) {
    TopkOfPlan pl{};
    const size_t rows = (size_t)std::max(S, 0), n = rows * (size_t)std::max(P, 1);
    Carve c;
    pl.o_key = c.take(n * sizeof(uint64_t));
    pl.o_sum = c.take(n * sizeof(bt_summary));
    pl.o_syms = c.take(rows * sizeof(SymDesc));
    pl.o_hist = c.take(4096 * sizeof(unsigned int));
    pl.o_state = c.take(4 * sizeof(unsigned long long));
    pl.o_counts = c.take(2 * sizeof(unsigned int));
    pl.o_above = c.take((size_t)kTopkCap * sizeof(unsigned long long));
    pl.o_cand = c.take((size_t)kTopkCap * sizeof(unsigned long long));
    pl.o_out = c.take(((size_t)kTopkMax + 1) * sizeof(bt_topk_rec));
    pl.staging_bytes = c.staging_bytes();
    return pl;
}

}
```

distributed-backtesting-exploration_amd/csrc/plan.h:

```cpp
#pragma once
#include "internal.h"

namespace bt {

constexpr int kCusFallback = 256;
constexpr size_t kCuLdsBytes = 160 * 1024;

struct AxisSpec {
    const int32_t* v;
    int32_t n;
    const char* what;
    int32_t lo, hi;
};
int config_axes(const bt_config& c, AxisSpec ax[4]);

std::string plan_grid(const bt_config& c, Grid& g);

struct LaunchPlan {
    int32_t G;
    int32_t burn_tiles;
    int32_t grid_y;
    int32_t block;
    size_t lds;
    int32_t dedicated, one_trip;
    int32_t ts;
    int32_t xw, lpw;
    int32_t split_grp;
    uint32_t wmap;
    size_t seg_slots;
    size_t pos_off, pos_bytes;
    size_t ema_doubles;
    bool topk_lds_free;
};

struct RunShape {
    int32_t n_sym, max_bars;
    bool parity;
    int32_t seg_req, burn_req;
    int cus;
};

LaunchPlan plan_launch(const Grid& g, const int32_t* ax0, const RunShape& r);

constexpr size_t kStagingAlign = 256;
struct Carve {
    size_t end = 0;
    size_t take(size_t bytes) {
        const size_t at = end;
        end = at + (bytes + kStagingAlign - 1) / kStagingAlign * kStagingAlign;
        return at;
    }
    size_t staging_bytes() const { return end > kStagingAlign ? end : kStagingAlign; }
};

constexpr size_t kReplayBudget = 256u << 20;
struct ReplayPlan {
    int64_t dcap;
    int64_t pitch;
    int32_t lanes_per_chunk, chunks;
    size_t o_lane, o_sum, o_trades, o_equity, o_pos;
    size_t staging_bytes;
};
ReplayPlan plan_replay(int32_t n, int32_t W, int32_t trade_cap, int64_t stride, bool equity, bool pos,
                       size_t budget_req = 0);

struct SurfacePlan {
    int32_t block;
    int32_t p_blocks;
    int32_t chunks;
    int32_t rows_per_chunk, rows_rem;
    int32_t p_tiles;
    int32_t fold_ways;
    size_t partial_bytes;
    size_t fold_bytes;
    size_t best_partial_bytes;
    size_t o_partial, o_fold, o_best_partial, o_agg, o_best, o_sum, o_ids;
    size_t staging_bytes;
};
SurfacePlan plan_surface(int32_t S, int32_t P, int cus, int32_t chunks_req, bool staged = false);

constexpr size_t kWalkfwdBudget = 256u << 20;
struct WalkfwdPlan {
    int32_t rows_per_chunk, chunks;
    int32_t sel_block;
    int32_t tiles;
    int64_t waves;
    double fill;
    size_t bounds_bytes, row_bytes;
    size_t staging_bytes;
    size_t o_rec, o_steps;
};
WalkfwdPlan plan_walkfwd(int32_t S, int32_t P, int32_t K, int32_t max_bars, int cus, int64_t budget_req = 0);

constexpr int32_t kPortfolioMaxReplicas = 64;
constexpr size_t kPortfolioAccBudget = 64u << 20;
struct PortfolioPlan {
    int32_t R;
    int32_t finish_block;
    int64_t pitch;
    int32_t tiles;
    double fill;
    size_t o_lanes, o_acc_pnl, o_acc_cnt, o_pnl, o_equity, o_long, o_short, o_sum;
    size_t acc_bytes;
    size_t out_bytes;
    size_t staging_bytes;
};
PortfolioPlan plan_portfolio(int32_t n, int32_t T, int cus, int32_t replicas_req = 0, size_t budget_req = 0);

constexpr int kGramWavesPerCu = 8;
constexpr int32_t kGramMinChunkBars = 512;
constexpr size_t kGramPartialBudget = 64u << 20;
constexpr size_t kGramStagingMax = 256u << 20;
struct GramPlan {
    int32_t nt, tiles;
    int32_t chunks, chunk_bars;
    int32_t fold_block;
    int64_t pitch;
    double fill;
    size_t o_lanes, o_d, o_partial, o_gram, o_sums;
    size_t d_bytes;
    size_t out_bytes;
    size_t staging_bytes;
};
GramPlan plan_gram(int32_t n, int32_t T, int cus, int32_t split_req = 0);

struct TopkOfPlan {
    size_t o_key, o_sum, o_syms;
    size_t o_hist, o_state, o_counts, o_above, o_cand, o_out;
    size_t staging_bytes;
};
TopkOfPlan plan_topk_of(int32_t S, int32_t P);

}
```

distributed-backtesting-exploration_amd/engine.py:

```python
from __future__ import annotations

import ctypes as C
import importlib.util
import os
import subprocess
import sys
from dataclasses import dataclass, field
from typing import Sequence

import numpy as np

PKG_DIR = os.path.dirname(os.path.abspath(__file__))
_bt_lib = os.path.normpath(os.environ.get("BT_LIB", "libbt.so"))
if _bt_lib.startswith("..") or os.path.isabs(_bt_lib):
    raise ImportError(f"BT_LIB={_bt_lib}: a path inside {PKG_DIR} (libbt.so or dev/NAME.so)")
LIB_PATH = os.path.join(PKG_DIR, _bt_lib)
CSRC = os.path.join(PKG_DIR, "csrc")
ABI_VERSION = 3
PIPE_SLOTS = 4

BT_SMA_CROSS, BT_EMA_OLS, BT_BOLL = 1, 2, 3
BT_FLAG_PARITY, BT_FLAG_TIMING = 1, 2
BT_DAILY, BT_MINUTE = 0, 1

SUMMARY_DTYPE = np.dtype([
    ("n_trades", "<i4"), ("status", "<i4"), ("pnl", "<i8"), ("mdd", "<i8"),
    ("exposure", "<i8"), ("sharpe", "<f8"), ("hash", "<u8"),
])
SUMS_DTYPE = np.dtype([("s1_lo", "<u8"), ("s1_hi", "<i8"), ("s2_lo", "<u8"), ("s2_hi", "<i8")])
TRADE_DTYPE = np.dtype([
    ("entry_bar", "<i4"), ("exit_bar", "<i4"), ("side", "<i4"), ("pad", "<i4"),
    ("entry_px", "<i8"), ("exit_px", "<i8"),
])
TOPK_DTYPE = np.dtype([("sharpe", "<f8"), ("sym", "<i4"), ("param", "<i4"), ("pnl", "<i8")])
LANE_DTYPE = np.dtype([("sym", "<i4"), ("param", "<i4")])
REPLAY_MAX = 4096
assert SUMMARY_DTYPE.itemsize == 48 and TOPK_DTYPE.itemsize == 24 and TRADE_DTYPE.itemsize == 32
assert LANE_DTYPE.itemsize == 8
PARAM_AGG_DTYPE = np.dtype([
    ("n_sym", "<i4"), ("n_traded", "<i4"), ("n_win", "<i4"), ("n_pos", "<i4"),
    ("trades", "<i8"), ("pnl", "<i8"), ("exposure", "<i8"), ("mdd_max", "<i8"),
    ("sharpe_max", "<f8"), ("sharpe_min", "<f8"), ("sym_max", "<i4"), ("sym_min", "<i4"),
    ("ss1_lo", "<u8"), ("ss1_hi", "<i8"), ("ss2_lo", "<u8"), ("ss2_hi", "<i8"),
])
assert PARAM_AGG_DTYPE.itemsize == 104
SURFACE_OF_MAX = 1 << 22
TOPK_OF_MAX = 1 << 22
FOLD_DTYPE = np.dtype([
    ("first_bar", "<i4"), ("n_bars", "<i4"), ("n_trades", "<i4"), ("status", "<i4"),
    ("pnl", "<i8"), ("mdd", "<i8"), ("exposure", "<i8"), ("sharpe", "<f8"),
    ("s1_lo", "<u8"), ("s1_hi", "<i8"), ("s2_lo", "<u8"), ("s2_hi", "<i8"),
])
WF_STEP_DTYPE = np.dtype([
    ("sym", "<i4"), ("fold", "<i4"), ("param", "<i4"), ("pad", "<i4"), ("train_sharpe", "<f8"),
    ("oos", FOLD_DTYPE),
])
assert FOLD_DTYPE.itemsize == 80 and WF_STEP_DTYPE.itemsize == 104
WALKFWD_FOLDS_MAX = 1 << 22
PF_LANE_DTYPE = np.dtype([("sym", "<i4"), ("param", "<i4"), ("from_bar", "<i4"), ("to_bar", "<i4")])
PF_SUMMARY_DTYPE = np.dtype([
    ("n_lanes", "<i4"), ("first_bar", "<i4"), ("n_bars", "<i4"), ("max_gross", "<i4"),
    ("pnl", "<i8"), ("mdd", "<i8"), ("exposure", "<i8"), ("sharpe", "<f8"),
    ("s1_lo", "<u8"), ("s1_hi", "<i8"), ("s2_lo", "<u8"), ("s2_hi", "<i8"),
])
assert PF_LANE_DTYPE.itemsize == 16 and PF_SUMMARY_DTYPE.itemsize == 80
PORTFOLIO_MAX = 1 << 20
PF_WHOLE = 2**31 - 1
WIDE_DTYPE = np.dtype([("lo", "<u8"), ("hi", "<i8")])
assert WIDE_DTYPE.itemsize == 16
COV_MAX = 2048


class BtError(RuntimeError):
    pass


class _Config(C.Structure):
    _fields_ = [
        ("strategy", C.c_int32),
        ("n_fast", C.c_int32), ("n_slow", C.c_int32),
        ("fast", C.POINTER(C.c_int32)), ("slow", C.POINTER(C.c_int32)),
        ("n_span", C.c_int32), ("n_ols", C.c_int32),
        ("span", C.POINTER(C.c_int32)), ("ols", C.POINTER(C.c_int32)),
        ("band_bps", C.c_int32),
        ("n_bwin", C.c_int32), ("n_k", C.c_int32), ("n_sl", C.c_int32), ("n_tp", C.c_int32),
        ("bwin", C.POINTER(C.c_int32)), ("k_num", C.POINTER(C.c_int32)),
        ("k_den", C.c_int32),
        ("sl_bps", C.POINTER(C.c_int32)), ("tp_bps", C.POINTER(C.c_int32)),
        ("annualization", C.c_int64),
        ("device", C.c_int32), ("topk", C.c_int32), ("flags", C.c_int32),
        ("host_threads", C.c_int32), ("trade_cap", C.c_int32),
        ("stream", C.c_void_p),
    ]


class _JobIn(C.Structure):
    _fields_ = [("id", C.c_char_p), ("file", C.c_void_p), ("len", C.c_size_t)]


class _JobOut(C.Structure):
    _fields_ = [("data", C.c_void_p), ("len", C.c_size_t), ("status", C.c_int32),
                ("n_bars", C.c_int32)]


class _BatchProfile(C.Structure):
    _fields_ = [("n_jobs", C.c_int64), ("n_failed", C.c_int64), ("payload_bytes", C.c_int64),
                ("payload_bytes_read", C.c_int64), ("bars", C.c_int64),
                ("host_ingest_ms", C.c_double), ("upload_ms", C.c_double),
                ("compute_ms", C.c_double), ("readback_ms", C.c_double),
                ("format_ms", C.c_double), ("total_ms", C.c_double)]


class _Stats(C.Structure):
    _fields_ = [("n_symbols", C.c_int64), ("n_params", C.c_int64), ("bar_evals", C.c_int64),
                ("trades", C.c_int64), ("errors", C.c_int64)]


_lib = None


def build(force: bool = False) -> str:
    if force or not os.path.exists(LIB_PATH):
        subprocess.run(["make", "-s", "-j8", "-C", CSRC], check=True)
    return LIB_PATH


def _one_hip_runtime():
    if "torch" in sys.modules:
        return
    if importlib.util.find_spec("torch") is not None:
        import torch


def lib():
    global _lib
    if _lib is not None:
        return _lib
    if not os.path.exists(LIB_PATH):
        raise BtError(f"{LIB_PATH} missing: run __graft_entry__.build() (no CPU fallback)")
    _one_hip_runtime()
    L = C.CDLL(LIB_PATH)
    P = C.c_void_p
    L.bt_engine_create.argtypes = [C.POINTER(_Config), C.c_char_p, C.c_size_t]
    L.bt_engine_create.restype = P
    L.bt_engine_destroy.argtypes = [P]
    L.bt_engine_destroy.restype = None
    L.bt_last_error.restype = C.c_char_p
    L.bt_abi_version.restype = C.c_int32
    L.bt_num_params.argtypes = [P]
    L.bt_set_segments.argtypes = [P, C.c_int32, C.c_int32]
    L.bt_last_segments.argtypes = [P, C.POINTER(C.c_int64)]
    L.bt_run_batch.argtypes = [P, C.c_size_t, C.POINTER(_JobIn), C.POINTER(_JobOut)]
    L.bt_job_out_free.argtypes = [C.POINTER(_JobOut), C.c_size_t]
    L.bt_job_out_free.restype = None
    L.bt_load_synthetic.argtypes = [P, C.c_uint64, C.c_int64, C.c_int32, C.c_int32, C.c_int32]
    L.bt_load_ohlc.argtypes = [P, C.c_int32, P, P, P, P, P, P]
    for f in ("bt_run", "bt_sync", "bt_reset_timing"):
        getattr(L, f).argtypes = [P]
    L.bt_read_summaries.argtypes = [P, P, C.c_size_t]
    L.bt_read_sums.argtypes = [P, P, C.c_size_t]
    L.bt_read_trades.argtypes = [P, P, C.c_size_t]
    L.bt_read_topk.argtypes = [P, P, C.c_int32]
    L.bt_read_stats.argtypes = [P, C.POINTER(_Stats)]
    L.bt_topk_fetch_async.argtypes = [P, C.c_int32]
    L.bt_topk_fetch_wait.argtypes = [P, C.c_int32, P, C.c_int32, C.POINTER(C.c_int64)]
    L.bt_read_close.argtypes = [P, C.c_int32, P, C.c_int32]
    L.bt_kernel_timing.argtypes = [P, C.POINTER(C.c_double), C.POINTER(C.c_int64),
                                   C.POINTER(C.c_char_p)]
    L.bt_merge_topk.argtypes = [P, C.c_size_t, C.c_int32, P]
    L.bt_i128_to_double.argtypes = [C.c_uint64, C.c_int64]
    L.bt_i128_to_double.restype = C.c_double
    L.bt_parse_csv.argtypes = [C.c_char_p, C.c_size_t, C.c_int32, P, P, P, C.c_char_p,
                               C.c_size_t]
    L.bt_parse_job.argtypes = L.bt_parse_csv.argtypes
    L.bt_encode_columns.argtypes = [P, P, P, P, P, C.c_int32, P, C.c_size_t]
    L.bt_encode_columns.restype = C.c_int64
    L.bt_gen_payload.argtypes = [C.c_uint64, C.c_int64, C.c_int32, C.c_int32, P, C.c_size_t]
    L.bt_gen_payload.restype = C.c_int64
    L.bt_last_batch_profile.argtypes = [P, C.POINTER(_BatchProfile)]
    L.bt_format_summaries.argtypes = [P, C.c_int32, P, C.c_size_t]
    L.bt_format_summaries.restype = C.c_int64
    _lib = L
    return L


_LATE_SYMBOLS = {
    "bt_comm_unique_id": (2, [C.c_void_p], C.c_int32),
    "bt_comm_create": (2, [C.c_void_p, C.c_int32, C.c_int32, C.c_int32, C.c_int32, C.c_char_p,
                           C.c_size_t], C.c_void_p),
    "bt_comm_destroy": (2, [C.c_void_p], None),
    "bt_exchange_async": (2, [C.c_void_p, C.c_void_p, C.c_int32], C.c_int32),
    "bt_exchange_wait": (2, [C.c_void_p, C.c_int32, C.c_void_p, C.c_int32, C.c_void_p], C.c_int32),
    "bt_exchange_message_bytes": (2, [C.c_int32], C.c_int64),
    "bt_exchange_merge": (3, [C.c_void_p, C.c_size_t, C.c_int32, C.c_int32, C.c_void_p, C.c_int32,
                              C.c_void_p], C.c_int32),
    "bt_replay": (3, [C.c_void_p, C.c_int32, C.c_void_p, C.c_int32, C.c_void_p, C.c_void_p,
                      C.c_void_p, C.c_void_p, C.c_void_p, C.c_int64], C.c_int32),
    "bt_surface": (3, [C.c_void_p, C.c_void_p, C.c_void_p], C.c_int32),
    "bt_surface_of": (3, [C.c_void_p, C.c_int32, C.c_int32, C.c_void_p, C.c_void_p, C.c_void_p,
                          C.c_void_p], C.c_int32),
    "bt_topk_of": (3, [C.c_void_p, C.c_int32, C.c_int32, C.c_void_p, C.c_void_p, C.c_int32, C.c_int32,
                       C.c_void_p], C.c_int32),
    "bt_set_surface_chunks": (3, [C.c_void_p, C.c_int32], C.c_int32),
    "bt_surface_host": (3, [C.c_int32, C.c_int32, C.c_void_p, C.c_void_p, C.c_void_p, C.c_void_p],
                        C.c_int32),
    "bt_surface_merge": (3, [C.c_void_p, C.c_int32, C.c_int32, C.c_void_p], C.c_int32),
    "bt_walk_forward": (3, [C.c_void_p, C.c_int32, C.c_void_p, C.c_int32, C.c_void_p, C.c_void_p,
                            C.c_void_p], C.c_int32),
    "bt_set_walkfwd_budget": (3, [C.c_void_p, C.c_int64], C.c_int32),
    "bt_walk_forward_host": (3, [C.c_int32, C.c_int32, C.c_int32, C.c_int32, C.c_void_p, C.c_void_p,
                                 C.c_int64, C.c_void_p, C.c_void_p], C.c_int32),
    "bt_portfolio": (3, [C.c_void_p, C.c_int32, C.c_void_p, C.c_int32, C.c_void_p, C.c_void_p, C.c_void_p,
                         C.c_void_p, C.c_void_p], C.c_int32),
    "bt_set_portfolio_replicas": (3, [C.c_void_p, C.c_int32], C.c_int32),
    "bt_portfolio_host": (3, [C.c_int32, C.c_void_p, C.c_void_p, C.c_void_p, C.c_int64, C.c_void_p, C.c_int32,
                              C.c_int64, C.c_void_p, C.c_void_p, C.c_void_p, C.c_void_p, C.c_void_p], C.c_int32),
    "bt_portfolio_merge": (3, [C.c_int32, C.c_int32, C.c_void_p, C.c_void_p, C.c_void_p, C.c_void_p, C.c_int64,
                               C.c_void_p, C.c_void_p, C.c_void_p, C.c_void_p, C.c_void_p], C.c_int32),
    "bt_covariance": (3, [C.c_void_p, C.c_int32, C.c_void_p, C.c_int32, C.c_int32, C.c_void_p, C.c_void_p,
                          C.c_void_p], C.c_int32),
    "bt_gram_of": (3, [C.c_void_p, C.c_int32, C.c_int32, C.c_void_p, C.c_void_p, C.c_void_p], C.c_int32),
    "bt_set_gram_split": (3, [C.c_void_p, C.c_int32], C.c_int32),
    "bt_covariance_host": (3, [C.c_int32, C.c_void_p, C.c_void_p, C.c_int64, C.c_int32, C.c_int32, C.c_void_p,
                               C.c_void_p, C.c_void_p], C.c_int32),
}
_late = {}


def sym(name: str):
    f = _late.get(name)
    if f is None:
        min_abi, argtypes, restype = _LATE_SYMBOLS[name]
        have = lib().bt_abi_version()
        if have < min_abi:
            raise BtError(f"{name}: {LIB_PATH} has ABI {have}, this binding needs ABI >= {min_abi}")
        f = getattr(lib(), name)
        f.argtypes, f.restype = argtypes, restype
        _late[name] = f
    return f


def _check(rc):
    if rc < 0:
        raise BtError(lib().bt_last_error().decode())
    return rc


def _arr(v) -> np.ndarray:
    return np.ascontiguousarray(np.asarray(v, dtype=np.int32))


@dataclass
class Grid:
    strategy: int
    axes: Sequence[Sequence[int]]
    band_bps: int = 20
    k_den: int = 2
    annualization: int = 252
    _keep: list = field(default_factory=list, repr=False)

    @property
    def n_params(self) -> int:
        n = 1
        for a in self.axes:
            n *= len(a)
        return n

    @staticmethod
    def sma(fast, slow, annualization=252):
        return Grid(BT_SMA_CROSS, [list(fast), list(slow)], annualization=annualization)

    @staticmethod
    def ema_ols(span, ols, band_bps=20, annualization=98280):
        return Grid(BT_EMA_OLS, [list(span), list(ols)], band_bps=band_bps,
                    annualization=annualization)

    @staticmethod
    def boll(win, k_num, sl_bps, tp_bps, k_den=2, annualization=98280):
        return Grid(BT_BOLL, [list(win), list(k_num), list(sl_bps), list(tp_bps)], k_den=k_den,
                    annualization=annualization)

    def param(self, p: int) -> dict:
        if self.strategy == BT_SMA_CROSS:
            return {"f": self.axes[0][p // len(self.axes[1])], "s": self.axes[1][p % len(self.axes[1])]}
        if self.strategy == BT_EMA_OLS:
            return {"n": self.axes[0][p // len(self.axes[1])], "w": self.axes[1][p % len(self.axes[1])],
                    "band_bps": self.band_bps}
        nk, nsl, ntp = (len(a) for a in self.axes[1:])
        return {"w": self.axes[0][p // (ntp * nsl * nk)], "k_num": self.axes[1][(p // (ntp * nsl)) % nk],
                "k_den": self.k_den, "sl": self.axes[2][(p // ntp) % nsl], "tp": self.axes[3][p % ntp]}

    def to_c(self, device=0, topk=0, flags=0, host_threads=0, trade_cap=0, stream=None) -> _Config:
        cfg = _Config()
        cfg.strategy = self.strategy
        arrs = [_arr(a) for a in self.axes]
        self._keep = arrs
        ptr = [a.ctypes.data_as(C.POINTER(C.c_int32)) for a in arrs]
        if self.strategy == BT_SMA_CROSS:
            cfg.n_fast, cfg.n_slow = len(arrs[0]), len(arrs[1])
            cfg.fast, cfg.slow = ptr
        elif self.strategy == BT_EMA_OLS:
            cfg.n_span, cfg.n_ols = len(arrs[0]), len(arrs[1])
            cfg.span, cfg.ols = ptr
            cfg.band_bps = self.band_bps
        else:
            cfg.n_bwin, cfg.n_k, cfg.n_sl, cfg.n_tp = (len(a) for a in arrs)
            cfg.bwin, cfg.k_num, cfg.sl_bps, cfg.tp_bps = ptr
            cfg.k_den = self.k_den
        cfg.annualization = self.annualization
        cfg.device, cfg.topk, cfg.flags = device, topk, flags
        cfg.host_threads, cfg.trade_cap = host_threads, trade_cap
        cfg.stream = stream
        return cfg


def config2_grid():
    return Grid.sma(range(4, 43, 2), range(50, 241, 10), annualization=252)


def config3_grid():
    return Grid.ema_ols([10, 20, 30, 60, 120, 240, 390, 780],
                        [15, 30, 60, 120, 240, 390, 780, 1560], band_bps=20, annualization=98280)


def config4_grid():
    return Grid.boll([10, 20, 30, 45, 60, 90, 120, 240], [3, 4, 5, 6], [50, 100],
                     [50, 100, 200, 400], k_den=2, annualization=98280)


def config5_grid():
    return Grid.sma(range(5, 161, 5), range(200, 6401, 200), annualization=98280)


def as_lanes(lanes) -> np.ndarray:
    a = lanes if isinstance(lanes, np.ndarray) else np.asarray(list(lanes))
    if a.dtype.names is not None:
        if not {"sym", "param"} <= set(a.dtype.names):
            raise ValueError("lane records need sym and param fields")
        a = a.reshape(-1)
    out = np.zeros(len(a), LANE_DTYPE)
    if a.dtype.names is not None:
        out["sym"], out["param"] = a["sym"], a["param"]
    elif len(a):
        if a.ndim != 2 or a.shape[1] != 2 or not np.issubdtype(a.dtype, np.integer):
            raise ValueError("lanes: top-k records, an (n, 2) integer array or a list of (sym, param) pairs")
        if a.min() < -2**31 or a.max() >= 2**31:
            raise ValueError("lanes: sym and param are int32")
        out["sym"], out["param"] = a[:, 0], a[:, 1]
    return out


@dataclass
class Replay:
    lanes: np.ndarray
    summaries: np.ndarray
    n_bars: np.ndarray
    trades: np.ndarray | None
    equity: np.ndarray | None
    pos: np.ndarray | None


@dataclass
class Surface:
    params: np.ndarray
    best: np.ndarray | None

    def _sum128(self, name) -> np.ndarray:
        return np.array([i128_to_double(int(r[name + "_lo"]), int(r[name + "_hi"])) for r in self.params],
                        np.float64)

    def mean_sharpe(self) -> np.ndarray:
        n = self.params["n_sym"].astype(np.float64)
        return np.divide(self._sum128("ss1") / 2.0**32, n, out=np.zeros(len(n)), where=n > 0)

    def std_sharpe(self) -> np.ndarray:
        n = self.params["n_sym"].astype(np.float64)
        m2 = np.divide(self._sum128("ss2") / 2.0**64, n, out=np.zeros(len(n)), where=n > 0)
        return np.sqrt(np.maximum(m2 - self.mean_sharpe() ** 2, 0.0))

    def win_rate(self) -> np.ndarray:
        n = self.params["n_sym"].astype(np.float64)
        return np.divide(self.params["n_win"].astype(np.float64), n, out=np.zeros(len(n)), where=n > 0)

    def rank(self, k=None, by="mean_sharpe") -> np.ndarray:
        derived = {"mean_sharpe": self.mean_sharpe, "std_sharpe": self.std_sharpe, "win_rate": self.win_rate}
        if by in derived:
            v = derived[by]()
        elif by in (self.params.dtype.names or ()):
            v = self.params[by]
        else:
            raise ValueError(f"rank by {by!r}: one of {sorted(derived)} or a field of PARAM_AGG_DTYPE")
        order = (len(v) - 1 - np.argsort(v[::-1], kind="stable"))[::-1]
        return order if k is None else order[:k]


def _surface_bufs(S, P, best):
    agg = np.zeros(max(P, 1), PARAM_AGG_DTYPE)
    rec = np.zeros(max(S, 1), TOPK_DTYPE) if best else None
    return agg, rec


def _as_matrix(summaries, sym_ids):
    m = np.ascontiguousarray(summaries, SUMMARY_DTYPE)
    if m.ndim != 2:
        raise ValueError("summaries: an S x P array of SUMMARY_DTYPE")
    ids = np.ascontiguousarray(np.asarray(sym_ids, np.int32))
    if ids.shape != (m.shape[0],):
        raise ValueError(f"sym_ids: {m.shape[0]} ids for {m.shape[0]} rows, got shape {ids.shape}")
    return m, ids


def surface_host(summaries, sym_ids, best=True) -> Surface:
    m, ids = _as_matrix(summaries, sym_ids)
    S, P = m.shape
    agg, rec = _surface_bufs(S, P, best)
    _check(sym("bt_surface_host")(S, P, m.ctypes.data if m.size else None, ids.ctypes.data if S else None,
                                  agg.ctypes.data, None if rec is None else rec.ctypes.data))
    return Surface(agg[:P], None if rec is None else rec[:S])


def merge_surfaces(parts) -> Surface:
    parts = list(parts)
    world = len(parts)
    P = len(parts[0].params) if parts else 0
    if any(len(s.params) != P for s in parts):
        raise ValueError("merge_surfaces: the surfaces hold different parameter counts")
    block = (np.ascontiguousarray(np.concatenate([s.params for s in parts]), PARAM_AGG_DTYPE) if parts
             else np.zeros(1, PARAM_AGG_DTYPE))
    out = np.zeros(max(P, 1), PARAM_AGG_DTYPE)
    _check(sym("bt_surface_merge")(block.ctypes.data, world, P, out.ctypes.data))
    best = (np.concatenate([s.best for s in parts]) if parts and all(s.best is not None for s in parts)
            else None)
    return Surface(out[:P], best)


@dataclass
class WalkForward:
    bounds: np.ndarray | None
    train: int
    steps: np.ndarray
    total: np.ndarray
    folds: np.ndarray | None

    def oos_sharpe(self) -> np.ndarray:
        return self.total["sharpe"].copy()

    def train_sharpe(self) -> np.ndarray:
        return self.steps["train_sharpe"].copy()


def _as_bounds(bounds) -> np.ndarray:
    b = np.asarray(list(bounds) if not isinstance(bounds, np.ndarray) else bounds)
    if b.ndim != 1 or not np.issubdtype(b.dtype, np.integer) or (len(b) and (b.min() < -2**31 or b.max() >= 2**31)):
        raise ValueError("bounds: a 1-D sequence of int32 bar indices")
    return np.ascontiguousarray(b, np.int32)


def walk_forward_host(folds, sym_ids, train: int = 1, annualization: int = 252) -> WalkForward:
    f = np.ascontiguousarray(folds, FOLD_DTYPE)
    if f.ndim != 3:
        raise ValueError("folds: an S x P x K array of FOLD_DTYPE")
    S, P, K = f.shape
    ids = np.ascontiguousarray(np.asarray(sym_ids, np.int32))
    if ids.shape != (S,):
        raise ValueError(f"sym_ids: {S} ids for {S} rows, got shape {ids.shape}")
    n_steps = max(K - max(train, 1), 0)
    steps = np.zeros((max(S, 1), max(n_steps, 1)), WF_STEP_DTYPE)
    total = np.zeros(max(S, 1), FOLD_DTYPE)
    _check(sym("bt_walk_forward_host")(S, P, K, train, f.ctypes.data if f.size else None,
                                       ids.ctypes.data if S else None, annualization, steps.ctypes.data,
                                       total.ctypes.data))
    steps = np.ascontiguousarray(steps.reshape(-1)[:S * n_steps]).reshape(S, n_steps)
    return WalkForward(None, train, steps, total[:S], f)


@dataclass
class Portfolio:
    pnl: np.ndarray
    equity: np.ndarray
    n_long: np.ndarray
    n_short: np.ndarray
    summary: np.ndarray
    annualization: int = 252

    def gross(self) -> np.ndarray:
        return self.n_long + self.n_short

    def net(self) -> np.ndarray:
        return self.n_long - self.n_short


def as_pf_lanes(lanes, windows=None) -> np.ndarray:
    if isinstance(lanes, np.ndarray) and lanes.dtype == PF_LANE_DTYPE:
        if windows is not None:
            raise ValueError("windows: the PF_LANE_DTYPE entries carry their own")
        return np.ascontiguousarray(lanes.reshape(-1))
    req = as_lanes(lanes)
    out = np.zeros(len(req), PF_LANE_DTYPE)
    out["sym"], out["param"] = req["sym"], req["param"]
    out["to_bar"] = PF_WHOLE
    if windows is not None:
        w = np.asarray(windows)
        if not np.issubdtype(w.dtype, np.integer) or w.shape not in ((2,), (len(req), 2)):
            raise ValueError("windows: one (from_bar, to_bar) pair or an (n, 2) integer array")
        if w.size and (w.min() < -2**31 or w.max() >= 2**31):
            raise ValueError("windows: from_bar and to_bar are int32")
        w = np.broadcast_to(w, (len(req), 2))
        out["from_bar"], out["to_bar"] = w[:, 0], w[:, 1]
    return out


def walk_forward_lanes(wf: WalkForward) -> np.ndarray:
    st = wf.steps.reshape(-1)
    st = st[st["param"] >= 0]
    out = np.zeros(len(st), PF_LANE_DTYPE)
    out["sym"], out["param"] = st["sym"], st["param"]
    out["from_bar"] = st["oos"]["first_bar"]
    out["to_bar"] = st["oos"]["first_bar"] + st["oos"]["n_bars"]
    return out


def _pf_bufs(T):
    T = max(int(T), 1)
    return (np.zeros(T, np.int64), np.zeros(T, np.int64), np.zeros(T, np.int32), np.zeros(T, np.int32),
            np.zeros(1, PF_SUMMARY_DTYPE))


def _pf_result(bufs, T, annualization) -> Portfolio:
    T = max(int(T), 0)
    pnl, eq, nl, ns, summ = bufs
    return Portfolio(pnl[:T], eq[:T], nl[:T], ns[:T], summ[0], int(annualization))


def portfolio_host(equity, pos, n_bars, windows=None, T=None, annualization: int = 252) -> Portfolio:
    eq = np.ascontiguousarray(equity, np.int64)
    ps = np.ascontiguousarray(pos, np.int8)
    nb = np.ascontiguousarray(np.asarray(n_bars, np.int32))
    if eq.ndim != 2 or ps.shape != eq.shape or nb.shape != (eq.shape[0],):
        raise ValueError("equity and pos: n x stride arrays, n_bars: n bar counts")
    n, stride = eq.shape
    req = as_pf_lanes(np.zeros((n, 2), np.int32), windows)
    if T is None:
        T = int(nb.max()) if n else 1
    bufs = _pf_bufs(T)
    _check(sym("bt_portfolio_host")(n, eq.ctypes.data if eq.size else None, ps.ctypes.data if ps.size else None,
                                    nb.ctypes.data if n else None, stride, req.ctypes.data if n else None, T,
                                    annualization, *(b.ctypes.data for b in bufs)))
    return _pf_result(bufs, T, annualization)


def merge_portfolios(parts) -> Portfolio:
    parts = list(parts)
    if not parts:
        raise ValueError("merge_portfolios: no parts")
    T, ann = len(parts[0].pnl), parts[0].annualization
    if any(len(p.pnl) != T or p.annualization != ann for p in parts):
        raise ValueError("merge_portfolios: the parts differ in their bars or annualization")
    pnl = np.ascontiguousarray(np.stack([p.pnl for p in parts]), np.int64)
    nl = np.ascontiguousarray(np.stack([p.n_long for p in parts]), np.int32)
    ns = np.ascontiguousarray(np.stack([p.n_short for p in parts]), np.int32)
    summ = np.ascontiguousarray(np.stack([p.summary for p in parts]), PF_SUMMARY_DTYPE)
    bufs = _pf_bufs(T)
    _check(sym("bt_portfolio_merge")(len(parts), T, pnl.ctypes.data, nl.ctypes.data, ns.ctypes.data, summ.ctypes.data,
                                     ann, *(b.ctypes.data for b in bufs)))
    return _pf_result(bufs, T, ann)


@dataclass
class Covariance:
    wide: np.ndarray
    sums: np.ndarray
    n_bars: int

    @property
    def gram(self) -> np.ndarray:
        out = np.empty(self.wide.shape, object)
        flat = out.reshape(-1)
        for k, (lo, hi) in enumerate(zip(self.wide["lo"].reshape(-1).tolist(), self.wide["hi"].reshape(-1).tolist())):
            flat[k] = (hi << 64) | lo
        return out

    @property
    def gram_f64(self) -> np.ndarray:
        out = np.empty(self.wide.shape, np.float64)
        flat = out.reshape(-1)
        for k, (lo, hi) in enumerate(zip(self.wide["lo"].reshape(-1).tolist(), self.wide["hi"].reshape(-1).tolist())):
            flat[k] = i128_to_double(lo, hi)
        return out

    def cov(self) -> np.ndarray:
        n = len(self.sums)
        if self.n_bars < 1:
            return np.zeros((n, n))
        T = float(self.n_bars)
        m = self.sums.astype(np.float64) / T
        return self.gram_f64 / T - np.outer(m, m)

    def vol(self) -> np.ndarray:
        v = np.diagonal(self.cov())
        return np.sqrt(np.where(v > 0, v, 0.0))

    def corr(self) -> np.ndarray:
        c = self.cov()
        v = np.diagonal(c)
        ok = v > 0
        den = np.sqrt(np.outer(np.where(ok, v, 1.0), np.where(ok, v, 1.0)))
        return np.where(np.outer(ok, ok), c / den, 0.0)

    def book_s2(self, weights=None) -> int:
        n = len(self.sums)
        w = [1] * n if weights is None else [int(x) for x in weights]
        if len(w) != n or (weights is not None and any(int(x) != x for x in weights)):
            raise ValueError("book_s2: one integer weight per lane")
        g = self.gram
        return sum(w[i] * w[j] * g[i, j] for i in range(n) for j in range(n))


def _window(window):
    if window is None:
        return 0, PF_WHOLE
    w = np.asarray(window)
    if w.shape != (2,) or not np.issubdtype(w.dtype, np.integer) or w.min() < -2**31 or w.max() >= 2**31:
        raise ValueError("window: one (from_bar, to_bar) pair of int32")
    return int(w[0]), int(w[1])


def _cov_result(n, wide, sums, T) -> Covariance:
    return Covariance(wide[:n * n].reshape(n, n), sums[:n], int(T))


def covariance_host(equity, n_bars, window=None) -> Covariance:
    eq = np.ascontiguousarray(equity, np.int64)
    nb = np.ascontiguousarray(np.asarray(n_bars, np.int32))
    if eq.ndim != 2 or nb.shape != (eq.shape[0],):
        raise ValueError("equity: an n x stride array, n_bars: n bar counts")
    n, stride = eq.shape
    frm, to = _window(window)
    wide, sums, T = np.zeros(max(n * n, 1), WIDE_DTYPE), np.zeros(max(n, 1), np.int64), C.c_int32(0)
    _check(sym("bt_covariance_host")(n, eq.ctypes.data if eq.size else None, nb.ctypes.data if n else None, stride,
                                     frm, to, wide.ctypes.data, sums.ctypes.data, C.addressof(T)))
    return _cov_result(n, wide, sums, T.value)


class Engine:

    def __init__(self, grid: Grid, device=0, topk=0, parity=False, timing=False,
                 trade_cap=0, host_threads=0, stream=None):
        self.grid = grid
        flags = (BT_FLAG_PARITY if parity else 0) | (BT_FLAG_TIMING if timing else 0)
        cfg = grid.to_c(device, topk, flags, host_threads, trade_cap, stream)
        err = C.create_string_buffer(512)
        h = lib().bt_engine_create(C.byref(cfg), err, 512)
        if not h:
            raise BtError(err.value.decode())
        self._h = h
        self.n_params = lib().bt_num_params(h)
        self.trade_cap = trade_cap
        self.n_symbols = 0
        self.topk = topk
        self._sym_bars = None

    def close(self):
        if getattr(self, "_h", None):
            lib().bt_engine_destroy(self._h)
            self._h = None

    __del__ = close

    def __enter__(self):
        return self

    def __exit__(self, *a):
        self.close()

    def load_synthetic(self, seed, sym_begin, n_sym, n_bars, freq=BT_DAILY):
        self._sym_bars = None
        _check(lib().bt_load_synthetic(self._h, seed & ((1 << 64) - 1), sym_begin, n_sym, n_bars, freq))
        self.n_symbols = n_sym
        self._sym_bars = (sym_begin, n_sym, n_bars)

    def load_ohlc(self, closes, highs=None, lows=None, sym_ids=None):
        bars = np.array([len(c) for c in closes], np.int32)
        offs = np.zeros(len(closes), np.int64)
        if len(closes):
            offs[1:] = np.cumsum(bars[:-1])
        cat = lambda xs: np.ascontiguousarray(np.concatenate([np.asarray(x, np.int32) for x in xs])) if len(xs) else np.zeros(1, np.int32)
        c = cat(closes)
        h = cat(highs) if highs is not None else None
        lo = cat(lows) if lows is not None else None
        ids = np.ascontiguousarray(np.arange(len(closes), dtype=np.int64) if sym_ids is None
                                   else np.asarray(sym_ids, np.int64))
        ptr = lambda a: None if a is None else a.ctypes.data
        self._sym_bars = None
        _check(lib().bt_load_ohlc(self._h, len(closes), ids.ctypes.data, bars.ctypes.data,
                                  offs.ctypes.data, ptr(h), ptr(lo), c.ctypes.data))
        self.n_symbols = len(closes)
        self._sym_bars = {}
        for i, b in zip(ids.astype(np.int32).tolist(), bars.tolist()):
            self._sym_bars.setdefault(i, b)

    def run(self):
        _check(lib().bt_run(self._h))

    def set_segments(self, segments: int, burn_tiles: int = 0) -> None:
        _check(lib().bt_set_segments(self._h, segments, burn_tiles))

    def last_segments(self, with_refixed: bool = False):
        n = C.c_int64(0)
        g = _check(lib().bt_last_segments(self._h, C.byref(n)))
        return (g, int(n.value)) if with_refixed else g

    def sync(self):
        _check(lib().bt_sync(self._h))

    def summaries(self) -> np.ndarray:
        n = self.n_symbols * self.n_params
        out = np.zeros(max(n, 1), SUMMARY_DTYPE)
        _check(lib().bt_read_summaries(self._h, out.ctypes.data, n))
        return out[:n].reshape(self.n_symbols, self.n_params)

    def sums(self) -> np.ndarray:
        n = self.n_symbols * self.n_params
        out = np.zeros(max(n, 1), SUMS_DTYPE)
        _check(lib().bt_read_sums(self._h, out.ctypes.data, n))
        return out[:n].reshape(self.n_symbols, self.n_params)

    def trades(self) -> np.ndarray:
        n = self.n_symbols * self.n_params * self.trade_cap
        out = np.zeros(max(n, 1), TRADE_DTYPE)
        _check(lib().bt_read_trades(self._h, out.ctypes.data, n))
        return out[:n].reshape(self.n_symbols, self.n_params, self.trade_cap)

    def read_topk(self, k=None) -> np.ndarray:
        k = k or self.topk
        out = np.zeros(k, TOPK_DTYPE)
        m = _check(lib().bt_read_topk(self._h, out.ctypes.data, k))
        return out[:m]

    def topk_fetch_async(self, slot: int) -> None:
        _check(lib().bt_topk_fetch_async(self._h, slot))

    def topk_fetch_wait(self, slot: int, k=None) -> tuple:
        k = k or self.topk
        out = np.zeros(k, TOPK_DTYPE)
        n = C.c_int64(0)
        m = _check(lib().bt_topk_fetch_wait(self._h, slot, out.ctypes.data, k, C.byref(n)))
        return out[:m], int(n.value)

    def replay(self, lanes, trade_cap: int = 0, curves: bool = False) -> Replay:
        req = as_lanes(lanes)
        n = len(req)
        f = sym("bt_replay")
        ptr = lambda a: None if a is None else a.ctypes.data
        summ = np.zeros(max(n, 1), SUMMARY_DTYPE)
        nb = np.zeros(max(n, 1), np.int32)
        tr = np.zeros((max(n, 1), trade_cap), TRADE_DTYPE) if trade_cap > 0 else None
        eq = ps = None
        stride = 0
        if curves:
            stride = self._replay_stride(f, req) if 0 < n <= REPLAY_MAX else 1
            eq = np.empty((max(n, 1), stride), np.int64)
            ps = np.empty((max(n, 1), stride), np.int8)
        _check(f(self._h, n, req.ctypes.data if n else None, trade_cap, summ.ctypes.data,
                 nb.ctypes.data, ptr(tr), ptr(eq), ptr(ps), stride))
        if curves:
            eq, ps = eq[:n], ps[:n]
            if n == 0:
                eq, ps = eq[:, :0], ps[:, :0]
        return Replay(req, summ[:n], nb[:n], None if tr is None else tr[:n], eq, ps)

    def _replay_stride(self, f, req) -> int:
        bars = self._sym_bars
        if isinstance(bars, tuple):
            begin, n_sym, b = bars
            if ((req["sym"] >= begin) & (req["sym"] < begin + n_sym)).all():
                return b
        elif isinstance(bars, dict):
            got = [bars.get(int(s)) for s in np.unique(req["sym"])]
            if None not in got:
                return max(got)
        summ = np.zeros(len(req), SUMMARY_DTYPE)
        nb = np.zeros(len(req), np.int32)
        _check(f(self._h, len(req), req.ctypes.data, 0, summ.ctypes.data, nb.ctypes.data, None, None,
                 None, 0))
        return int(nb.max())

    def surface(self, best: bool = True) -> Surface:
        f = sym("bt_surface")
        S = self.stats()["n_symbols"]
        agg, rec = _surface_bufs(S, self.n_params, best)
        _check(f(self._h, agg.ctypes.data, None if rec is None else rec.ctypes.data))
        return Surface(agg[:self.n_params], None if rec is None else rec[:S])

    def surface_of(self, summaries, sym_ids, best: bool = True) -> Surface:
        m, ids = _as_matrix(summaries, sym_ids)
        S, P = m.shape
        agg, rec = _surface_bufs(S, P, best)
        _check(sym("bt_surface_of")(self._h, S, P, m.ctypes.data if m.size else None,
                                    ids.ctypes.data if S else None, agg.ctypes.data,
                                    None if rec is None else rec.ctypes.data))
        return Surface(agg[:P], None if rec is None else rec[:S])

    def topk_of(self, summaries, sym_ids, k: int, lds_free_hist: bool = False) -> np.ndarray:
        m, ids = _as_matrix(summaries, sym_ids)
        S, P = m.shape
        out = np.zeros(max(k, 1), TOPK_DTYPE)
        n = _check(sym("bt_topk_of")(self._h, S, P, m.ctypes.data if m.size else None,
                                     ids.ctypes.data if S else None, k, int(bool(lds_free_hist)),
                                     out.ctypes.data))
        return out[:n]

    def set_surface_chunks(self, n: int) -> None:
        _check(sym("bt_set_surface_chunks")(self._h, n))

    def walk_forward(self, bounds, train: int = 1, folds: bool = False) -> WalkForward:
        b = _as_bounds(bounds)
        K = len(b) - 1
        S = self.stats()["n_symbols"]
        n_steps = max(K - max(train, 1), 0)
        steps = np.zeros(max(S * n_steps, 1), WF_STEP_DTYPE)
        total = np.zeros(max(S, 1), FOLD_DTYPE)
        want = K >= 2
        rec = None
        if folds:
            if S * self.n_params * max(K, 0) > WALKFWD_FOLDS_MAX:
                raise BtError(f"bt_walk_forward: S*P*K = {S}*{self.n_params}*{K} exceeds 2^22 fold records")
            rec = np.zeros(max(S * self.n_params * max(K, 0), 1), FOLD_DTYPE)
        _check(sym("bt_walk_forward")(self._h, K, b.ctypes.data if len(b) else None, train,
                                      None if rec is None else rec.ctypes.data,
                                      steps.ctypes.data if want else None, total.ctypes.data if want else None))
        return WalkForward(b, train, steps[:S * n_steps].reshape(S, n_steps), total[:S],
                           None if rec is None else rec[:S * self.n_params * K].reshape(S, self.n_params, K))

    def set_walkfwd_budget(self, nbytes: int) -> None:
        _check(sym("bt_set_walkfwd_budget")(self._h, nbytes))

    def portfolio(self, lanes, windows=None, n_bars=None) -> Portfolio:
        req = as_pf_lanes(lanes, windows)
        T = self._longest(req["sym"]) if n_bars is None else int(n_bars)
        bufs = _pf_bufs(T)
        _check(sym("bt_portfolio")(self._h, len(req), req.ctypes.data if len(req) else None, T,
                                   *(b.ctypes.data for b in bufs)))
        return _pf_result(bufs, T, self.grid.annualization)

    def _longest(self, syms) -> int:
        bars = self._sym_bars
        if isinstance(bars, tuple):
            return bars[2]
        if isinstance(bars, dict) and bars:
            return max(bars.values())
        ids = np.unique(np.asarray(syms, np.int32))
        longest = 1
        for i in range(0, len(ids), REPLAY_MAX):
            part = np.zeros(len(ids[i:i + REPLAY_MAX]), LANE_DTYPE)
            part["sym"] = ids[i:i + REPLAY_MAX]
            longest = max(longest, self._replay_stride(sym("bt_replay"), part))
        return longest

    def set_portfolio_replicas(self, r: int) -> None:
        _check(sym("bt_set_portfolio_replicas")(self._h, r))

    def covariance(self, lanes, window=None) -> Covariance:
        req = as_lanes(lanes)
        n = len(req)
        frm, to = _window(window)
        wide, sums, T = np.zeros(max(n * n, 1), WIDE_DTYPE), np.zeros(max(n, 1), np.int64), C.c_int32(0)
        _check(sym("bt_covariance")(self._h, n, req.ctypes.data if n else None, frm, to, wide.ctypes.data,
                                    sums.ctypes.data, C.addressof(T)))
        return _cov_result(n, wide, sums, T.value)

    def gram_of(self, d) -> Covariance:
        a = np.asarray(d)
        if a.ndim != 2 or not np.issubdtype(a.dtype, np.integer):
            raise ValueError("gram_of: an n x T integer array")
        if a.size and (a.min() < -2**31 or a.max() >= 2**31):
            raise ValueError("gram_of: the increments are int32")
        a = np.ascontiguousarray(a, np.int32)
        n, T = a.shape
        wide, sums = np.zeros(max(n * n, 1), WIDE_DTYPE), np.zeros(max(n, 1), np.int64)
        _check(sym("bt_gram_of")(self._h, n, T, a.ctypes.data if a.size else None, wide.ctypes.data,
                                 sums.ctypes.data))
        return _cov_result(n, wide, sums, T)

    def set_gram_split(self, k: int) -> None:
        _check(sym("bt_set_gram_split")(self._h, k))

    def stats(self) -> dict:
        st = _Stats()
        _check(lib().bt_read_stats(self._h, C.byref(st)))
        return {f: getattr(st, f) for f, _ in _Stats._fields_}

    def close_column(self, sym_index, n) -> np.ndarray:
        out = np.zeros(n, np.int32)
        _check(lib().bt_read_close(self._h, sym_index, out.ctypes.data, n))
        return out

    def kernel_timing(self):
        ms, n, name = C.c_double(), C.c_int64(), C.c_char_p()
        _check(lib().bt_kernel_timing(self._h, C.byref(ms), C.byref(n), C.byref(name)))
        return ms.value, n.value, name.value.decode()

    def reset_timing(self):
        _check(lib().bt_reset_timing(self._h))

    def run_batch(self, jobs: Sequence[tuple]) -> list:
        n = len(jobs)
        jin = (_JobIn * max(n, 1))()
        keep = []
        for i, (jid, data) in enumerate(jobs):
            b = bytes(data)
            idb = jid.encode() if isinstance(jid, str) else bytes(jid)
            keep += [b, idb]
            jin[i].id = idb
            jin[i].file = C.cast(C.c_char_p(b), C.c_void_p)
            jin[i].len = len(b)
        jout = (_JobOut * max(n, 1))()
        self._sym_bars = None
        try:
            _check(lib().bt_run_batch(self._h, n, jin, jout))
            res = [(jout[i].status, C.string_at(jout[i].data, jout[i].len).decode()) for i in range(n)]
        finally:
            lib().bt_job_out_free(jout, n)
        return res

    def batch_profile(self) -> dict:
        pr = _BatchProfile()
        _check(lib().bt_last_batch_profile(self._h, C.byref(pr)))
        return {f: getattr(pr, f) for f, _ in _BatchProfile._fields_}


class Comm:

    ID_BYTES = 128

    @staticmethod
    def unique_id() -> bytes:
        buf = C.create_string_buffer(Comm.ID_BYTES)
        _check(sym("bt_comm_unique_id")(buf))
        return buf.raw

    def __init__(self, uid: bytes, rank: int, world: int, device: int, k: int):
        if len(uid) != Comm.ID_BYTES:
            raise ValueError("RCCL unique id must be 128 bytes")
        err = C.create_string_buffer(512)
        self._uid = C.create_string_buffer(bytes(uid), Comm.ID_BYTES)
        h = sym("bt_comm_create")(self._uid, rank, world, device, k, err, 512)
        if not h:
            raise BtError(err.value.decode())
        self._h, self.k, self.world = h, k, world

    def exchange_async(self, engine: "Engine", slot: int) -> None:
        _check(sym("bt_exchange_async")(self._h, engine._h, slot))

    def exchange_wait(self, slot: int, k=None) -> tuple:
        k = k or self.k
        out = np.zeros(k, TOPK_DTYPE)
        cnt = np.zeros(2, np.int64)
        m = _check(sym("bt_exchange_wait")(self._h, slot, out.ctypes.data, k, cnt.ctypes.data))
        return out[:m], [int(cnt[0]), int(cnt[1])]

    def close(self):
        if getattr(self, "_h", None):
            sym("bt_comm_destroy")(self._h)
            self._h = None

    __del__ = close


def merge_topk(records: np.ndarray, k: int) -> np.ndarray:
    recs = np.ascontiguousarray(records, TOPK_DTYPE)
    out = np.zeros(max(k, 1), TOPK_DTYPE)
    m = _check(lib().bt_merge_topk(recs.ctypes.data if len(recs) else None, len(recs), k,
                                   out.ctypes.data))
    return out[:m]


def exchange_message(records: np.ndarray, k_msg: int, bar_evals: int, trades: int) -> bytes:
    n = len(records)
    size = _check(sym("bt_exchange_message_bytes")(k_msg))
    buf = np.zeros(size, np.uint8)
    buf[:4] = np.frombuffer(np.int32(n).tobytes(), np.uint8)
    rec = TOPK_DTYPE.itemsize
    if n:
        buf[rec:rec * (1 + n)] = np.frombuffer(np.ascontiguousarray(records, TOPK_DTYPE).tobytes(), np.uint8)
    buf[rec * (k_msg + 1):] = np.frombuffer(np.array([bar_evals, trades], np.int64).tobytes(), np.uint8)
    return buf.tobytes()


def exchange_merge(block: bytes, world: int, k_msg: int, k: int) -> tuple:
    raw = np.frombuffer(block, np.uint8)
    need = world * _check(sym("bt_exchange_message_bytes")(k_msg))
    if len(raw) != need:
        raise BtError(f"exchange block holds {len(raw)} bytes, expected {need} "
                      f"(world {world} x message of k_msg {k_msg})")
    out = np.zeros(max(k, 1), TOPK_DTYPE)
    cnt = np.zeros(2, np.int64)
    m = _check(sym("bt_exchange_merge")(raw.ctypes.data, len(raw), world, k_msg, out.ctypes.data,
                                        k, cnt.ctypes.data))
    return out[:m], [int(cnt[0]), int(cnt[1])]


def format_summaries(rows: np.ndarray) -> str:
    rows = np.ascontiguousarray(rows, SUMMARY_DTYPE)
    cap = _check(lib().bt_format_summaries(None, len(rows), None, 0))
    buf = C.create_string_buffer(max(cap, 1))
    n = _check(lib().bt_format_summaries(rows.ctypes.data if len(rows) else None, len(rows), buf, cap))
    return buf.raw[:n].decode()


def i128_to_double(lo: int, hi: int) -> float:
    return lib().bt_i128_to_double(lo & ((1 << 64) - 1), hi)


def parse_csv(data: bytes, cap=1 << 22):
    cap = int(cap)
    h, lo, c = (np.empty(cap, np.int32) for _ in range(3))
    err = C.create_string_buffer(256)
    n = lib().bt_parse_job(data, len(data), cap, h.ctypes.data, lo.ctypes.data, c.ctypes.data,
                           err, 256)
    if n < 0:
        raise ValueError(err.value.decode())
    return h[:n].copy(), lo[:n].copy(), c[:n].copy()
```

include/bt.h:

```cpp
#ifndef BT_H
#define BT_H
#include <stddef.h>
#include <stdint.h>

#ifdef __cplusplus
extern "C" {
#endif

#define BT_ABI_VERSION 3

typedef struct bt_engine bt_engine;

enum bt_strategy { BT_SMA_CROSS = 1, BT_EMA_OLS = 2, BT_BOLL = 3 };

enum bt_flags {
    BT_FLAG_PARITY = 1,
    BT_FLAG_TIMING = 2,
};

enum bt_freq { BT_DAILY = 0, BT_MINUTE = 1 };

typedef struct bt_config {
    int32_t strategy;
    int32_t n_fast, n_slow;
    const int32_t* fast;
    const int32_t* slow;
    int32_t n_span, n_ols;
    const int32_t* span;
    const int32_t* ols;
    int32_t band_bps;
    int32_t n_bwin, n_k, n_sl, n_tp;
    const int32_t* bwin;
    const int32_t* k_num;
    int32_t k_den;
    const int32_t* sl_bps;
    const int32_t* tp_bps;
    int64_t annualization;
    int32_t device;
    int32_t topk;
    int32_t flags;
    int32_t host_threads;
    int32_t trade_cap;
    void* stream;
} bt_config;

typedef struct bt_job_in {
    const char* id;
    const uint8_t* file;
    size_t len;
} bt_job_in;

typedef struct bt_job_out {
    char* data;
    size_t len;
    int32_t status;
    int32_t n_bars;
} bt_job_out;

typedef struct bt_summary {
    int32_t n_trades;
    int32_t status;
    int64_t pnl;
    int64_t mdd;
    int64_t exposure;
    double sharpe;
    uint64_t hash;
} bt_summary;

typedef struct bt_trade {
    int32_t entry_bar, exit_bar, side, pad;
    int64_t entry_px, exit_px;
} bt_trade;

typedef struct bt_sums {
    uint64_t s1_lo;
    int64_t s1_hi;
    uint64_t s2_lo;
    int64_t s2_hi;
} bt_sums;

typedef struct bt_topk_rec {
    double sharpe;
    int32_t sym;
    int32_t param;
    int64_t pnl;
} bt_topk_rec;

typedef struct bt_stats {
    int64_t n_symbols;
    int64_t n_params;
    int64_t bar_evals;
    int64_t trades;
    int64_t errors;
} bt_stats;

bt_engine* bt_engine_create(const bt_config* cfg, char* err, size_t errlen);
void bt_engine_destroy(bt_engine* e);
const char* bt_last_error(void);
int32_t bt_abi_version(void);
int32_t bt_num_params(const bt_engine* e);
int32_t bt_set_segments(bt_engine* e, int32_t segments, int32_t burn_tiles);
int32_t bt_last_segments(bt_engine* e, int64_t* refixed_blocks);

typedef struct bt_batch_profile {
    int64_t n_jobs, n_failed;
    int64_t payload_bytes;
    int64_t payload_bytes_read;
    int64_t bars;
    double host_ingest_ms;
    double upload_ms;
    double compute_ms;
    double readback_ms;
    double format_ms;
    double total_ms;
} bt_batch_profile;

int32_t bt_run_batch(bt_engine* e, size_t n, const bt_job_in* jobs, bt_job_out* outs);
void bt_job_out_free(bt_job_out* outs, size_t n);
int32_t bt_last_batch_profile(bt_engine* e, bt_batch_profile* out);

int32_t bt_load_synthetic(bt_engine* e, uint64_t seed, int64_t sym_begin, int32_t n_sym,
                          int32_t n_bars, int32_t freq);
int32_t bt_load_ohlc(bt_engine* e, int32_t n_sym, const int64_t* sym_ids, const int32_t* bars,
                     const int64_t* row_off, const int32_t* h, const int32_t* l,
                     const int32_t* c);
int32_t bt_run(bt_engine* e);
int32_t bt_sync(bt_engine* e);
int32_t bt_read_summaries(bt_engine* e, bt_summary* out, size_t n);
int32_t bt_read_sums(bt_engine* e, bt_sums* out, size_t n);
int32_t bt_read_trades(bt_engine* e, bt_trade* out, size_t n);
int32_t bt_read_topk(bt_engine* e, bt_topk_rec* out, int32_t k);
int32_t bt_read_stats(bt_engine* e, bt_stats* out);
#define BT_PIPE_SLOTS 4
int32_t bt_topk_fetch_async(bt_engine* e, int32_t slot);
int32_t bt_topk_fetch_wait(bt_engine* e, int32_t slot, bt_topk_rec* out, int32_t k,
                           int64_t* n_trades);
int32_t bt_read_close(bt_engine* e, int32_t sym_index, int32_t* out, int32_t n);
typedef struct bt_lane {
    int32_t sym;
    int32_t param;
} bt_lane;
#define BT_REPLAY_MAX 4096
int32_t bt_replay(bt_engine* e, int32_t n, const bt_lane* lanes, int32_t trade_cap,
                  bt_summary* sum,
                  int32_t* n_bars,
                  bt_trade* trades,
                  int64_t* equity,
                  int8_t* pos,
                  int64_t stride);
typedef struct bt_param_agg {
    int32_t n_sym, n_traded, n_win, n_pos;
    int64_t trades, pnl, exposure, mdd_max;
    double  sharpe_max, sharpe_min;
    int32_t sym_max, sym_min;
    uint64_t ss1_lo; int64_t ss1_hi; uint64_t ss2_lo; int64_t ss2_hi;
} bt_param_agg;

int32_t bt_surface(bt_engine* e, bt_param_agg* agg, bt_topk_rec* best);
int32_t bt_surface_of(bt_engine* e, int32_t S, int32_t P, const bt_summary* sum,
                      const int32_t* sym_ids, bt_param_agg* agg, bt_topk_rec* best);
int32_t bt_topk_of(bt_engine* e, int32_t S, int32_t P, const bt_summary* sum,
                   const int32_t* sym_ids, int32_t k, int32_t lds_free_hist, bt_topk_rec* out);
int32_t bt_set_surface_chunks(bt_engine* e, int32_t chunks);
int32_t bt_surface_host(int32_t S, int32_t P, const bt_summary* sum, const int32_t* sym_ids,
                        bt_param_agg* agg, bt_topk_rec* best);
int32_t bt_surface_merge(const bt_param_agg* in, int32_t world, int32_t P, bt_param_agg* out);
typedef struct bt_fold {
    int32_t first_bar, n_bars, n_trades, status;
    int64_t pnl, mdd, exposure;
    double  sharpe;
    uint64_t s1_lo; int64_t s1_hi; uint64_t s2_lo; int64_t s2_hi;
} bt_fold;
typedef struct bt_wf_step {
    int32_t sym, fold, param, pad;
    double  train_sharpe;
    bt_fold oos;
} bt_wf_step;
int32_t bt_walk_forward(bt_engine* e, int32_t K, const int32_t* bounds , int32_t train,
                        bt_fold* folds, bt_wf_step* steps, bt_fold* total);
int32_t bt_set_walkfwd_budget(bt_engine* e, int64_t bytes);
int32_t bt_walk_forward_host(int32_t S, int32_t P, int32_t K, int32_t train, const bt_fold* folds,
                             const int32_t* sym_ids, int64_t annualization, bt_wf_step* steps,
                             bt_fold* total);
typedef struct bt_pf_lane {
    int32_t sym;
    int32_t param;
    int32_t from_bar, to_bar;
} bt_pf_lane;
typedef struct bt_pf_summary {
    int32_t n_lanes;
    int32_t first_bar, n_bars;
    int32_t max_gross;
    int64_t pnl;
    int64_t mdd;
    int64_t exposure;
    double  sharpe;
    uint64_t s1_lo; int64_t s1_hi; uint64_t s2_lo; int64_t s2_hi;
} bt_pf_summary;
#define BT_PORTFOLIO_MAX (1 << 20)
int32_t bt_portfolio(bt_engine* e, int32_t n, const bt_pf_lane* lanes, int32_t T,
                     int64_t* pnl,
                     int64_t* equity,
                     int32_t* n_long,
                     int32_t* n_short,
                     bt_pf_summary* summary);
int32_t bt_set_portfolio_replicas(bt_engine* e, int32_t r);
int32_t bt_portfolio_host(int32_t n, const int64_t* equity, const int8_t* pos, const int32_t* n_bars,
                          int64_t stride, const bt_pf_lane* lanes, int32_t T, int64_t annualization,
                          int64_t* out_pnl, int64_t* out_equity, int32_t* out_long, int32_t* out_short,
                          bt_pf_summary* summary);
int32_t bt_portfolio_merge(int32_t world, int32_t T, const int64_t* pnl, const int32_t* n_long,
                           const int32_t* n_short, const bt_pf_summary* summaries, int64_t annualization,
                           int64_t* out_pnl, int64_t* out_equity, int32_t* out_long, int32_t* out_short,
                           bt_pf_summary* summary);
typedef struct bt_wide {
    uint64_t lo;
    int64_t hi;
} bt_wide;
#define BT_COV_MAX 2048
int32_t bt_covariance(bt_engine* e, int32_t n, const bt_lane* lanes, int32_t from_bar, int32_t to_bar,
                      bt_wide* gram,
                      int64_t* sums,
                      int32_t* T_out);
int32_t bt_gram_of(bt_engine* e, int32_t n, int32_t T, const int32_t* d, bt_wide* gram, int64_t* sums);
int32_t bt_set_gram_split(bt_engine* e, int32_t k);
int32_t bt_covariance_host(int32_t n, const int64_t* equity, const int32_t* n_bars, int64_t stride,
                           int32_t from_bar, int32_t to_bar, bt_wide* gram, int64_t* sums, int32_t* T_out);
int32_t bt_kernel_timing(bt_engine* e, double* total_ms, int64_t* launches, const char** name);
int32_t bt_reset_timing(bt_engine* e);
int32_t bt_read_debug(bt_engine* e, uint64_t* out, int32_t n);

int32_t bt_merge_topk(const bt_topk_rec* in, size_t n, int32_t k, bt_topk_rec* out);

#define BT_COMM_ID_BYTES 128
typedef struct bt_comm bt_comm;
int32_t bt_comm_unique_id(uint8_t* out);
bt_comm* bt_comm_create(const uint8_t* id, int32_t rank, int32_t world, int32_t device, int32_t k,
                        char* err, size_t errlen);
void bt_comm_destroy(bt_comm* c);
int32_t bt_exchange_async(bt_comm* c, bt_engine* e, int32_t slot);
int32_t bt_exchange_wait(bt_comm* c, int32_t slot, bt_topk_rec* out, int32_t k,
                         int64_t* counters);
int64_t bt_exchange_message_bytes(int32_t k_msg);
int32_t bt_exchange_merge(const uint8_t* block, size_t block_bytes, int32_t world, int32_t k_msg,
                          bt_topk_rec* out, int32_t k, int64_t* counters);

int64_t bt_format_summaries(const bt_summary* r, int32_t P, char* out, size_t cap);
double bt_i128_to_double(uint64_t lo, int64_t hi);
int32_t bt_parse_csv(const uint8_t* buf, size_t len, int32_t cap, int32_t* h, int32_t* l,
                     int32_t* c, char* err, size_t errlen);
int32_t bt_parse_job(const uint8_t* buf, size_t len, int32_t cap, int32_t* h, int32_t* l,
                     int32_t* c, char* err, size_t errlen);

int64_t bt_encode_columns(const int32_t* o, const int32_t* h, const int32_t* l, const int32_t* c,
                          const int64_t* v, int32_t n, uint8_t* out, size_t cap);
int64_t bt_gen_payload(uint64_t seed, int64_t sym, int32_t bars, int32_t freq, uint8_t* out,
                       size_t cap);

#ifdef __cplusplus
}
#endif
#endif
```

Measured before the change: 4755 billion bar-evals/s.

## Alternate back-to-back runs across two streams so consecutive kernels overlap

Adds a second owned stream and sends odd-numbered runs to it, so a run's tail can overlap the next run's head when the grid needs several rounds of blocks per CU. Every other use of the main stream now goes through a helper that waits on the last run-stream event, and the run stream waits on main-stream work through a recorded event. Per-buffer done events and timing logic are extended to handle two in-flight launches. A new ABI call can turn the overlap off. This adds cross-stream event bookkeeping and ordering risk in exchange for less tail idle time between runs.

```diff
diff --git a/distributed-backtesting-exploration_amd/csrc/analysis.cpp b/distributed-backtesting-exploration_amd/csrc/analysis.cpp
--- a/distributed-backtesting-exploration_amd/csrc/analysis.cpp
+++ b/distributed-backtesting-exploration_amd/csrc/analysis.cpp
@@ -53,26 +53,26 @@
     out.pitch = pl.pitch;
     auto fetch = [&](void* dst, size_t dst_pitch, const void* src, size_t src_pitch, size_t m) {
         if (dst_pitch == src_pitch) {
-            HIPCHK(hipMemcpyAsync(dst, src, m * src_pitch, hipMemcpyDeviceToHost, e->stream));
+            HIPCHK(hipMemcpyAsync(dst, src, m * src_pitch, hipMemcpyDeviceToHost, main_stream(e)));
             return;
         }
-        HIPCHK(hipMemcpy2DAsync(dst, dst_pitch, src, src_pitch, src_pitch, m, hipMemcpyDeviceToHost, e->stream));
+        HIPCHK(hipMemcpy2DAsync(dst, dst_pitch, src, src_pitch, src_pitch, m, hipMemcpyDeviceToHost, main_stream(e)));
         for (size_t i = 0; i < m; ++i)
             memset(static_cast<uint8_t*>(dst) + i * dst_pitch + src_pitch, 0, dst_pitch - src_pitch);
     };
     for_chunks((size_t)n, (size_t)pl.lanes_per_chunk, [&](size_t i0, size_t m) {
-        HIPCHK(hipMemcpyAsync(d_lanes, req.data() + i0, m * sizeof(ReplayLane), hipMemcpyHostToDevice, e->stream));
-        if (dcap) HIPCHK(hipMemsetAsync(out.trades, 0, m * dcap * sizeof(bt_trade), e->stream));
-        if (equity) HIPCHK(hipMemsetAsync(out.equity, 0, m * pitch * 8, e->stream));
-        if (pos) HIPCHK(hipMemsetAsync(out.pos, 0, m * pitch, e->stream));
-        HIPCHK(launch_replay(d_lanes, (int32_t)m, e->d_h.p, e->d_l.p, e->d_c.p, e->grid, out, e->stream));
-        HIPCHK(hipMemcpyAsync(sum + i0, out.sum, m * sizeof(bt_summary), hipMemcpyDeviceToHost, e->stream));
+        HIPCHK(hipMemcpyAsync(d_lanes, req.data() + i0, m * sizeof(ReplayLane), hipMemcpyHostToDevice, main_stream(e)));
+        if (dcap) HIPCHK(hipMemsetAsync(out.trades, 0, m * dcap * sizeof(bt_trade), main_stream(e)));
+        if (equity) HIPCHK(hipMemsetAsync(out.equity, 0, m * pitch * 8, main_stream(e)));
+        if (pos) HIPCHK(hipMemsetAsync(out.pos, 0, m * pitch, main_stream(e)));
+        HIPCHK(launch_replay(d_lanes, (int32_t)m, e->d_h.p, e->d_l.p, e->d_c.p, e->grid, out, main_stream(e)));
+        HIPCHK(hipMemcpyAsync(sum + i0, out.sum, m * sizeof(bt_summary), hipMemcpyDeviceToHost, main_stream(e)));
         if (dcap)
             fetch(trades + i0 * (size_t)trade_cap, (size_t)trade_cap * sizeof(bt_trade), out.trades,
                   dcap * sizeof(bt_trade), m);
         if (equity) fetch(equity + i0 * (size_t)stride, (size_t)stride * 8, out.equity, pitch * 8, m);
         if (pos) fetch(pos + i0 * (size_t)stride, (size_t)stride, out.pos, pitch, m);
-        HIPCHK(hipStreamSynchronize(e->stream));
+        HIPCHK(hipStreamSynchronize(main_stream(e)));
     });
     if (n_bars)
         for (int32_t i = 0; i < n; ++i) n_bars[i] = req[i].bars;
@@ -88,13 +88,13 @@
     w.best_partial = at<bt_topk_rec>(base, pl.o_best_partial);
     w.agg = agg ? at<bt_param_agg>(base, pl.o_agg) : nullptr;
     w.best = best ? at<bt_topk_rec>(base, pl.o_best) : nullptr;
-    HIPCHK(launch_surface(d_sum, d_ids, id_stride, S, P, pl, w, e->stream));
+    HIPCHK(launch_surface(d_sum, d_ids, id_stride, S, P, pl, w, main_stream(e)));
     const size_t n_agg = (size_t)P * sizeof(bt_param_agg), n_best = (size_t)S * sizeof(bt_topk_rec);
     const size_t lo = agg ? pl.o_agg : pl.o_best, hi = best && S > 0 ? pl.o_best + n_best : pl.o_agg + n_agg;
     if (hi <= lo) return;
     e->h_surface.ensure(hi - lo);
-    HIPCHK(hipMemcpyAsync(e->h_surface.p, base + lo, hi - lo, hipMemcpyDeviceToHost, e->stream));
-    HIPCHK(hipStreamSynchronize(e->stream));
+    HIPCHK(hipMemcpyAsync(e->h_surface.p, base + lo, hi - lo, hipMemcpyDeviceToHost, main_stream(e)));
+    HIPCHK(hipStreamSynchronize(main_stream(e)));
     if (agg) memcpy(agg, e->h_surface.p + (pl.o_agg - lo), n_agg);
     if (best && S > 0) memcpy(best, e->h_surface.p + (pl.o_best - lo), n_best);
 }
@@ -128,8 +128,8 @@
     bt_summary* d_sum = at<bt_summary>(base, pl.o_sum);
     int32_t* d_ids = at<int32_t>(base, pl.o_ids);
     if (S > 0) {
-        HIPCHK(hipMemcpyAsync(d_sum, sum, (size_t)S * (size_t)P * sizeof(bt_summary), hipMemcpyHostToDevice, e->stream));
-        HIPCHK(hipMemcpyAsync(d_ids, ids, (size_t)S * sizeof(int32_t), hipMemcpyHostToDevice, e->stream));
+        HIPCHK(hipMemcpyAsync(d_sum, sum, (size_t)S * (size_t)P * sizeof(bt_summary), hipMemcpyHostToDevice, main_stream(e)));
+        HIPCHK(hipMemcpyAsync(d_ids, ids, (size_t)S * sizeof(int32_t), hipMemcpyHostToDevice, main_stream(e)));
     }
     surface_launch(e, pl, base, d_sum, d_ids, 1, S, P, agg, best);
     return 0;
@@ -156,15 +156,15 @@
     const TopkWork w{at<unsigned int>(base, pl.o_hist),      at<unsigned long long>(base, pl.o_state),
                      at<unsigned int>(base, pl.o_counts),    at<unsigned long long>(base, pl.o_above),
                      at<unsigned long long>(base, pl.o_cand), kTopkCap, d_out + 1, reinterpret_cast<int32_t*>(d_out)};
-    HIPCHK(hipMemcpyAsync(d_key, key.data(), n * sizeof(uint64_t), hipMemcpyHostToDevice, e->stream));
-    HIPCHK(hipMemcpyAsync(d_sum, sum, n * sizeof(bt_summary), hipMemcpyHostToDevice, e->stream));
-    HIPCHK(hipMemcpyAsync(d_syms, syms.data(), (size_t)S * sizeof(SymDesc), hipMemcpyHostToDevice, e->stream));
-    HIPCHK(hipMemsetAsync(d_out, 0, ((size_t)kTopkMax + 1) * sizeof(bt_topk_rec), e->stream));
-    HIPCHK(launch_topk_init(w, e->stream));
-    HIPCHK(launch_topk(d_key, d_sum, d_syms, (int64_t)n, P, k, w, e->stream, lds_free_hist != 0));
+    HIPCHK(hipMemcpyAsync(d_key, key.data(), n * sizeof(uint64_t), hipMemcpyHostToDevice, main_stream(e)));
+    HIPCHK(hipMemcpyAsync(d_sum, sum, n * sizeof(bt_summary), hipMemcpyHostToDevice, main_stream(e)));
+    HIPCHK(hipMemcpyAsync(d_syms, syms.data(), (size_t)S * sizeof(SymDesc), hipMemcpyHostToDevice, main_stream(e)));
+    HIPCHK(hipMemsetAsync(d_out, 0, ((size_t)kTopkMax + 1) * sizeof(bt_topk_rec), main_stream(e)));
+    HIPCHK(launch_topk_init(w, main_stream(e)));
+    HIPCHK(launch_topk(d_key, d_sum, d_syms, (int64_t)n, P, k, w, main_stream(e), lds_free_hist != 0));
     std::vector<bt_topk_rec> got((size_t)k + 1);
-    HIPCHK(hipMemcpyAsync(got.data(), d_out, got.size() * sizeof(bt_topk_rec), hipMemcpyDeviceToHost, e->stream));
-    HIPCHK(hipStreamSynchronize(e->stream));
+    HIPCHK(hipMemcpyAsync(got.data(), d_out, got.size() * sizeof(bt_topk_rec), hipMemcpyDeviceToHost, main_stream(e)));
+    HIPCHK(hipStreamSynchronize(main_stream(e)));
     int32_t count;
     memcpy(&count, &got[0], sizeof count);
     if (count < 0 || count > k) refuse(fn, "the device wrote a count of " + std::to_string(count));
@@ -190,7 +190,7 @@
     const bool select = steps || total;
     const int32_t n_steps = select ? walkfwd_steps(K, train) : 0;
     const size_t row_recs = (size_t)K * (size_t)P;
-    HIPCHK(hipMemcpyAsync(base, bounds, ((size_t)K + 1) * sizeof(int32_t), hipMemcpyHostToDevice, e->stream));
+    HIPCHK(hipMemcpyAsync(base, bounds, ((size_t)K + 1) * sizeof(int32_t), hipMemcpyHostToDevice, main_stream(e)));
     WfArgs a{};
     a.bounds = at<const int32_t>(base, 0);
     a.rec = at<bt_fold>(base, pl.o_rec);
@@ -203,16 +203,16 @@
     for_chunks((size_t)S, (size_t)pl.rows_per_chunk, [&](size_t r0, size_t m) {
         a.syms = e->d_syms.p + r0;
         a.n_rows = (int32_t)m;
-        HIPCHK(hipMemsetAsync(a.rec, 0, m * row_recs * sizeof(bt_fold), e->stream));
-        HIPCHK(launch_wf_walk(a, e->d_h.p, e->d_l.p, e->d_c.p, e->grid, e->stream));
+        HIPCHK(hipMemsetAsync(a.rec, 0, m * row_recs * sizeof(bt_fold), main_stream(e)));
+        HIPCHK(launch_wf_walk(a, e->d_h.p, e->d_l.p, e->d_c.p, e->grid, main_stream(e)));
         if (select) {
-            HIPCHK(launch_wf_select(a, e->grid, pl, e->stream));
+            HIPCHK(launch_wf_select(a, e->grid, pl, main_stream(e)));
             HIPCHK(hipMemcpyAsync(st + r0 * (size_t)n_steps, a.steps, m * (size_t)n_steps * sizeof(bt_wf_step),
-                                  hipMemcpyDeviceToHost, e->stream));
+                                  hipMemcpyDeviceToHost, main_stream(e)));
         }
         if (folds)
-            HIPCHK(hipMemcpyAsync(h_rec.data(), a.rec, m * row_recs * sizeof(bt_fold), hipMemcpyDeviceToHost, e->stream));
-        HIPCHK(hipStreamSynchronize(e->stream));
+            HIPCHK(hipMemcpyAsync(h_rec.data(), a.rec, m * row_recs * sizeof(bt_fold), hipMemcpyDeviceToHost, main_stream(e)));
+        HIPCHK(hipStreamSynchronize(main_stream(e)));
         if (folds)
             for (size_t r = 0; r < m; ++r)
                 for (size_t k = 0; k < (size_t)K; ++k)
@@ -251,11 +251,11 @@
     w.n_short = at<int32_t>(base, pl.o_short);
     w.sum = at<bt_pf_summary>(base, pl.o_sum);
     if (m > 0)
-        HIPCHK(hipMemcpyAsync(d_lanes, rs.req.data(), (size_t)m * sizeof(PfLane), hipMemcpyHostToDevice, e->stream));
-    HIPCHK(hipMemsetAsync(base + pl.o_acc_pnl, 0, pl.acc_bytes, e->stream));
-    HIPCHK(launch_portfolio(d_lanes, m, e->d_h.p, e->d_l.p, e->d_c.p, e->grid, w, pl, e->stream));
-    HIPCHK(hipMemcpyAsync(e->h_portfolio.p, base + pl.o_pnl, pl.out_bytes, hipMemcpyDeviceToHost, e->stream));
-    HIPCHK(hipStreamSynchronize(e->stream));
+        HIPCHK(hipMemcpyAsync(d_lanes, rs.req.data(), (size_t)m * sizeof(PfLane), hipMemcpyHostToDevice, main_stream(e)));
+    HIPCHK(hipMemsetAsync(base + pl.o_acc_pnl, 0, pl.acc_bytes, main_stream(e)));
+    HIPCHK(launch_portfolio(d_lanes, m, e->d_h.p, e->d_l.p, e->d_c.p, e->grid, w, pl, main_stream(e)));
+    HIPCHK(hipMemcpyAsync(e->h_portfolio.p, base + pl.o_pnl, pl.out_bytes, hipMemcpyDeviceToHost, main_stream(e)));
+    HIPCHK(hipStreamSynchronize(main_stream(e)));
     const uint8_t* h = e->h_portfolio.p;
     const size_t bars = (size_t)T;
     if (pnl) memcpy(pnl, h, bars * 8);
@@ -281,8 +281,8 @@
 
 void gram_fetch(bt_engine* e, uint8_t* base, const GramPlan& pl, int32_t n, bt_wide* gram, int64_t* sums) {
     e->h_gram.ensure(pl.out_bytes);
-    HIPCHK(hipMemcpyAsync(e->h_gram.p, base + pl.o_gram, pl.out_bytes, hipMemcpyDeviceToHost, e->stream));
-    HIPCHK(hipStreamSynchronize(e->stream));
+    HIPCHK(hipMemcpyAsync(e->h_gram.p, base + pl.o_gram, pl.out_bytes, hipMemcpyDeviceToHost, main_stream(e)));
+    HIPCHK(hipStreamSynchronize(main_stream(e)));
     if (gram) memcpy(gram, e->h_gram.p, (size_t)n * (size_t)n * sizeof(bt_wide));
     if (sums) memcpy(sums, e->h_gram.p + (pl.o_sums - pl.o_gram), (size_t)n * sizeof(int64_t));
 }
@@ -311,10 +311,10 @@
     uint8_t* base = enter(e, pl.staging_bytes);
     ReplayLane* d_lanes = at<ReplayLane>(base, pl.o_lanes);
     const GramWork w = gram_work(base, pl, n, T);
-    HIPCHK(hipMemcpyAsync(d_lanes, req.data(), (size_t)n * sizeof(ReplayLane), hipMemcpyHostToDevice, e->stream));
-    HIPCHK(hipMemsetAsync(base + pl.o_d, 0, pl.d_bytes, e->stream));
-    HIPCHK(launch_gram_walk(d_lanes, e->d_h.p, e->d_l.p, e->d_c.p, e->grid, w, from_bar, from_bar + T, e->stream));
-    HIPCHK(launch_gram(w, pl, false, e->stream));
+    HIPCHK(hipMemcpyAsync(d_lanes, req.data(), (size_t)n * sizeof(ReplayLane), hipMemcpyHostToDevice, main_stream(e)));
+    HIPCHK(hipMemsetAsync(base + pl.o_d, 0, pl.d_bytes, main_stream(e)));
+    HIPCHK(launch_gram_walk(d_lanes, e->d_h.p, e->d_l.p, e->d_c.p, e->grid, w, from_bar, from_bar + T, main_stream(e)));
+    HIPCHK(launch_gram(w, pl, false, main_stream(e)));
     gram_fetch(e, base, pl, n, gram, sums);
     return 0;
 }
@@ -336,10 +336,10 @@
     if (!why.empty()) refuse(fn, why);
     uint8_t* base = enter(e, pl.staging_bytes);
     const GramWork w = gram_work(base, pl, n, T);
-    HIPCHK(hipMemsetAsync(base + pl.o_d, 0, pl.d_bytes, e->stream));
+    HIPCHK(hipMemsetAsync(base + pl.o_d, 0, pl.d_bytes, main_stream(e)));
     HIPCHK(hipMemcpy2DAsync(w.D, (size_t)pl.pitch * sizeof(int32_t), d, (size_t)T * sizeof(int32_t),
-                            (size_t)T * sizeof(int32_t), (size_t)n, hipMemcpyHostToDevice, e->stream));
-    HIPCHK(launch_gram(w, pl, true, e->stream));
+                            (size_t)T * sizeof(int32_t), (size_t)n, hipMemcpyHostToDevice, main_stream(e)));
+    HIPCHK(launch_gram(w, pl, true, main_stream(e)));
     gram_fetch(e, base, pl, n, gram, sums);
     return 0;
 }
diff --git a/distributed-backtesting-exploration_amd/csrc/engine.cpp b/distributed-backtesting-exploration_amd/csrc/engine.cpp
--- a/distributed-backtesting-exploration_amd/csrc/engine.cpp
+++ b/distributed-backtesting-exploration_amd/csrc/engine.cpp
@@ -80,7 +80,7 @@
     e->d_syms.ensure(std::max<size_t>(1, n_sym));
     if (n_sym)
         HIPCHK(hipMemcpyAsync(e->d_syms.p, e->syms.data(), n_sym * sizeof(SymDesc),
-                              hipMemcpyHostToDevice, e->stream));
+                              hipMemcpyHostToDevice, main_stream(e)));
     const size_t r = std::max<int64_t>(1, rows);
     e->d_c.ensure(r);
     if (has_hl(e)) {
@@ -126,38 +126,52 @@
         e->d_cand.ensure(kTopkCap);
         e->d_top.ensure(kTopkMax + 1);
         e->h_top.ensure(kTopkMax + 1);
-        HIPCHK(launch_topk_init(topk_work(e), e->stream));
+        HIPCHK(launch_topk_init(topk_work(e), main_stream(e)));
         e->topk_ready = true;
     }
+}
+
+void run_stream_follows_main(bt_engine* e) {
+    if (!e->main_dirty || !e->rstream) return;
+    HIPCHK(hipEventRecord(e->ev_main, e->stream));
+    HIPCHK(hipStreamWaitEvent(e->rstream, e->ev_main, 0));
+    e->main_dirty = false;
 }
 
 void run_impl(bt_engine* e) {
     activate(e);
     ensure_outputs(e);
     const int32_t S = (int32_t)e->syms.size();
+    const bool parity = (e->cfg.flags & BT_FLAG_PARITY) != 0;
+    const LaunchPlan pl = plan_launch(e->grid, e->ax[0].data(),
+                                      RunShape{S, e->max_bars, parity, e->seg_req, e->burn_req, e->cus,
+                                               e->stream.owned, e->overlap_on});
     const int64_t run = e->nrun++;
     const int b = (int)(run & 1);
     e->cur = b;
+    const int slot = (int)(run % kNtrRing);
+    if (slot % (kNtrRing / 2) == 0) {
+        HIPCHK(hipMemsetAsync(e->d_ntr_ring.p + slot, 0, (kNtrRing / 2) * sizeof(unsigned long long),
+                              main_stream(e)));
+        run_stream_follows_main(e);
+    }
+    const bool on_run = pl.overlap && b == 1;
+    if (on_run) run_stream_follows_main(e);
+    const hipStream_t st = on_run ? (hipStream_t)e->rstream : pl.overlap ? (hipStream_t)e->stream : main_stream(e);
     if (e->tdone_armed[b] && hipEventQuery(e->ev_tdone[b]) != hipSuccess)
-        HIPCHK(hipStreamWaitEvent(e->stream, e->ev_tdone[b], 0));
+        HIPCHK(hipStreamWaitEvent(st, e->ev_tdone[b], 0));
     Out out{};
     out.sum = e->d_sum[b].p;
     out.key = e->d_key[b].p;
-    const bool parity = (e->cfg.flags & BT_FLAG_PARITY) != 0;
     out.sums = parity ? e->d_sums.p : nullptr;
     out.trades = parity ? e->d_trades.p : nullptr;
     out.trade_cap = parity ? e->cfg.trade_cap : 0;
-    const int slot = (int)(run % kNtrRing);
-    if (slot % (kNtrRing / 2) == 0)
-        HIPCHK(hipMemsetAsync(e->d_ntr_ring.p + slot, 0, (kNtrRing / 2) * sizeof(unsigned long long),
-                              e->stream));
     e->ntr[b] = e->d_ntr_ring.p + slot;
     out.n_trades = e->ntr[b];
     out.dbg = nullptr;
     if (BT_ABL(e->grid, 64)) {
         e->d_dbg.ensure(kDbgSlots + 8 * kDbgBlocks);
-        HIPCHK(hipMemsetAsync(e->d_dbg.p, 0, (kDbgSlots + 8 * kDbgBlocks) * sizeof(unsigned long long),
-                              e->stream));
+        HIPCHK(hipMemsetAsync(e->d_dbg.p, 0, (kDbgSlots + 8 * kDbgBlocks) * sizeof(unsigned long long), st));
         out.dbg = e->d_dbg.p;
     }
     const bool timing = (e->cfg.flags & BT_FLAG_TIMING) != 0;
@@ -169,10 +183,8 @@
         }
         ev.first.ensure(0);
         ev.second.ensure(0);
-        HIPCHK(hipEventRecord(ev.first, e->stream));
-    }
-    const LaunchPlan pl = plan_launch(e->grid, e->ax[0].data(),
-                                      RunShape{S, e->max_bars, parity, e->seg_req, e->burn_req, e->cus});
+        HIPCHK(hipEventRecord(ev.first, st));
+    }
     SegArgs sg{nullptr, nullptr, nullptr, nullptr, pl.G, pl.burn_tiles};
     if (pl.G > 1) {
         e->d_seg.ensure(pl.seg_slots);
@@ -183,32 +195,34 @@
             sg.ema = e->d_segema.p;
         }
         e->d_refixed.ensure(1);
-        HIPCHK(hipMemsetAsync(e->d_refixed.p, 0, sizeof(unsigned long long), e->stream));
+        HIPCHK(hipMemsetAsync(e->d_refixed.p, 0, sizeof(unsigned long long), st));
         sg.refixed = e->d_refixed.p;
     }
     e->seg_last = pl.G;
     hipError_t err;
     switch (e->cfg.strategy) {
         case BT_SMA_CROSS:
-            err = launch_sma(e->d_syms.p, S, e->d_c.p, e->grid, out, parity, sg, pl, e->stream);
+            err = launch_sma(e->d_syms.p, S, e->d_c.p, e->grid, out, parity, sg, pl, st);
             break;
         case BT_EMA_OLS:
-            err = launch_ema_ols(e->d_syms.p, S, e->d_c.p, e->grid, out, parity, sg, pl, e->stream);
+            err = launch_ema_ols(e->d_syms.p, S, e->d_c.p, e->grid, out, parity, sg, pl, st);
             break;
         default:
             err = launch_boll(e->d_syms.p, S, e->d_h.p, e->d_l.p, e->d_c.p, e->grid, out, parity, sg, pl,
-                              e->stream);
+                              st);
             break;
     }
     HIPCHK(err);
-    hipEvent_t kdone = e->ev_kdone;
+    hipEvent_t kdone = e->ev_kdone[on_run];
     if (timing) {
-        HIPCHK(hipEventRecord(ev.second, e->stream));
+        HIPCHK(hipEventRecord(ev.second, st));
         kdone = ev.second;
         e->ev_pending.push_back(std::move(ev));
-    }
+    } else if (e->cfg.topk > 0 || on_run) {
+        HIPCHK(hipEventRecord(kdone, st));
+    }
+    if (on_run) e->r_last = kdone;
     if (e->cfg.topk > 0) {
-        if (!timing) HIPCHK(hipEventRecord(kdone, e->stream));
         HIPCHK(hipStreamWaitEvent(e->tstream, kdone, 0));
         HIPCHK(launch_topk(e->d_key[b].p, e->d_sum[b].p, e->d_syms.p, (int64_t)S * e->P, e->P,
                            e->cfg.topk, topk_work(e), e->tstream, pl.topk_lds_free));
@@ -221,11 +235,18 @@
 void drain_timing(bt_engine* e) {
     for (auto& ev : e->ev_pending) {
         HIPCHK(hipEventSynchronize(ev.second));
+        if (e->r_last == ev.second.ev) e->r_last = nullptr;
         float ms = 0.f;
         HIPCHK(hipEventElapsedTime(&ms, ev.first, ev.second));
+        if (e->ev_last.second) {
+            float since = 0.f;
+            HIPCHK(hipEventElapsedTime(&since, e->ev_last.second, ev.second));
+            ms = std::min(ms, std::max(since, 0.f));
+            e->ev_pool.push_back(std::move(e->ev_last));
+        }
         e->kernel_ms += ms;
         e->launches += 1;
-        e->ev_pool.push_back(std::move(ev));
+        e->ev_last = std::move(ev);
     }
     e->ev_pending.clear();
 }
@@ -262,17 +283,17 @@
         for (Event& ev : e->ev_batch) ev.ensure(0);
         e->h_sum.ensure(nres);
         set_dataset(e, std::move(syms), rows);
-        HIPCHK(hipEventRecord(e->ev_batch[0], e->stream));
+        HIPCHK(hipEventRecord(e->ev_batch[0], main_stream(e)));
         int32_t* dst[3] = {e->d_c.p, e->d_h.p, e->d_l.p};
         for (int k = 0; k < ncol; ++k)
             HIPCHK(hipMemcpyAsync(dst[k], e->h_stage[k].p, (size_t)rows * 4, hipMemcpyHostToDevice,
-                                  e->stream));
-        HIPCHK(hipEventRecord(e->ev_batch[1], e->stream));
+                                  main_stream(e)));
+        HIPCHK(hipEventRecord(e->ev_batch[1], main_stream(e)));
         run_impl(e);
-        HIPCHK(hipEventRecord(e->ev_batch[2], e->stream));
+        HIPCHK(hipEventRecord(e->ev_batch[2], main_stream(e)));
         HIPCHK(hipMemcpyAsync(e->h_sum.p, e->d_sum[e->cur].p, nres * sizeof(bt_summary),
-                              hipMemcpyDeviceToHost, e->stream));
-        HIPCHK(hipEventRecord(e->ev_batch[3], e->stream));
+                              hipMemcpyDeviceToHost, main_stream(e)));
+        HIPCHK(hipEventRecord(e->ev_batch[3], main_stream(e)));
         sync_all(e);
         float ms = 0.f;
         HIPCHK(hipEventElapsedTime(&ms, e->ev_batch[0], e->ev_batch[1]));
@@ -334,8 +355,10 @@
         e->stream.borrow((hipStream_t)cfg->stream);
     else
         e->stream.create();
+    if (e->stream.owned) e->rstream.create();
     e->tstream.create();
-    e->ev_kdone.ensure(hipEventDisableTiming);
+    for (Event& ev : e->ev_kdone) ev.ensure(hipEventDisableTiming);
+    e->ev_main.ensure(hipEventDisableTiming);
     for (Event& ev : e->ev_tdone) ev.ensure(hipEventDisableTiming);
     upload_grid(e.get());
 #ifdef BT_PROFILING
@@ -367,6 +390,14 @@
         if (!e || segments < 0 || segments > 64 || burn_tiles < 0) throw HipFail{"bad arguments"};
         e->seg_req = segments;
         e->burn_req = burn_tiles;
+        return 0;
+    })
+}
+
+int32_t bt_set_run_overlap(bt_engine* e, int32_t on) {
+    ABI_GUARD(-1, {
+        if (!e) throw HipFail{"bt_set_run_overlap: null engine"};
+        e->overlap_on = on != 0;
         return 0;
     })
 }
@@ -400,7 +431,7 @@
         for (int32_t s = 0; s < n_sym; ++s) ids[s] = sym_begin + s;
         layout(e, n_sym, bars.data(), ids.data());
         HIPCHK(launch_gen(e->d_syms.p, n_sym, seed, freq, nullptr, has_hl(e) ? e->d_h.p : nullptr,
-                          has_hl(e) ? e->d_l.p : nullptr, e->d_c.p, e->stream));
+                          has_hl(e) ? e->d_l.p : nullptr, e->d_c.p, main_stream(e)));
         sync_all(e);
         return 0;
     })
@@ -428,7 +459,7 @@
                 for (int32_t s = 0; s < n_sym; ++s)
                     memcpy(e->h_stage[k].p + e->syms[s].off, src[k] + row_off[s], (size_t)bars[s] * 4);
                 HIPCHK(hipMemcpyAsync(dst[k], e->h_stage[k].p, (size_t)e->rows * 4,
-                                      hipMemcpyHostToDevice, e->stream));
+                                      hipMemcpyHostToDevice, main_stream(e)));
             }
             sync_all(e);
         }
diff --git a/distributed-backtesting-exploration_amd/csrc/engine_state.h b/distributed-backtesting-exploration_amd/csrc/engine_state.h
--- a/distributed-backtesting-exploration_amd/csrc/engine_state.h
+++ b/distributed-backtesting-exploration_amd/csrc/engine_state.h
@@ -17,13 +17,17 @@
     std::vector<int32_t> ax[4];
     Grid grid{};
     int32_t P = 0;
-    Stream tstream, stream;
+    Stream tstream, rstream, stream;
     ~EngineState() {
         if (!stream) return;
         (void)hipSetDevice(cfg.device);
         (void)hipStreamSynchronize(stream);
+        if (rstream) (void)hipStreamSynchronize(rstream);
         if (tstream) (void)hipStreamSynchronize(tstream);
     }
+    hipEvent_t r_last = nullptr;
+    bool main_dirty = false;
+    bool overlap_on = true;
     DevBuf<int32_t> d_axes[4];
     DevBuf<int32_t> d_kwin;
     DevBuf<double> d_krecip;
@@ -46,7 +50,8 @@
     DevBuf<double> d_segema;
     DevBuf<unsigned long long> d_refixed;
     DevBuf<unsigned long long> d_dbg;
-    Event ev_kdone;
+    Event ev_kdone[2];
+    Event ev_main;
     Event ev_tdone[2];
     bool tdone_armed[2] = {false, false};
     DevBuf<unsigned int> d_hist, d_counts;
@@ -59,6 +64,7 @@
     bool topk_ready = false;
     bool ran = false;
     std::vector<std::pair<Event, Event>> ev_pending, ev_pool;
+    std::pair<Event, Event> ev_last;
     double kernel_ms = 0.0;
     int64_t launches = 0;
     PinnedBuf<int32_t> h_stage[3];
@@ -88,7 +94,18 @@
 
 inline void sync_all(bt_engine* e) {
     HIPCHK(hipStreamSynchronize(e->stream));
+    if (e->rstream) HIPCHK(hipStreamSynchronize(e->rstream));
+    e->r_last = nullptr;
     if (e->tstream) HIPCHK(hipStreamSynchronize(e->tstream));
+}
+
+inline hipStream_t main_stream(bt_engine* e) {
+    if (e->r_last) {
+        if (hipEventQuery(e->r_last) != hipSuccess) HIPCHK(hipStreamWaitEvent(e->stream, e->r_last, 0));
+        e->r_last = nullptr;
+    }
+    e->main_dirty = true;
+    return e->stream;
 }
 
 template <class T>
diff --git a/distributed-backtesting-exploration_amd/csrc/plan.cpp b/distributed-backtesting-exploration_amd/csrc/plan.cpp
--- a/distributed-backtesting-exploration_amd/csrc/plan.cpp
+++ b/distributed-backtesting-exploration_amd/csrc/plan.cpp
@@ -274,6 +274,13 @@
     pl.seg_slots = seg_records(pl, g, r);
 }
 
+bool several_rounds(const LaunchPlan& pl, const RunShape& r) {
+    const long long waves = std::max(1, pl.block / 64);
+    const long long by_lds = pl.lds ? (long long)(kCuLdsBytes / pl.lds) : 32;
+    const long long per_cu = std::max<long long>(1, std::min<long long>(by_lds, 32 / waves));
+    return (long long)r.n_sym * pl.grid_y > per_cu * std::max(r.cus, 1);
+}
+
 }
 
 LaunchPlan plan_launch(const Grid& g, const int32_t* ax0, const RunShape& r) {
@@ -285,6 +292,7 @@
         case BT_EMA_OLS: plan_ema(g, ax0, r, pl); break;
         default: plan_boll(g, r, pl); break;
     }
+    pl.overlap = pl.G == 1 && !r.parity && !BT_ABL(g, 64) && r.own_stream && r.overlap_on && several_rounds(pl, r);
     return pl;
 }
 
diff --git a/distributed-backtesting-exploration_amd/csrc/plan.h b/distributed-backtesting-exploration_amd/csrc/plan.h
--- a/distributed-backtesting-exploration_amd/csrc/plan.h
+++ b/distributed-backtesting-exploration_amd/csrc/plan.h
@@ -31,6 +31,7 @@
     size_t pos_off, pos_bytes;
     size_t ema_doubles;
     bool topk_lds_free;
+    bool overlap;
 };
 
 struct RunShape {
@@ -38,6 +39,8 @@
     bool parity;
     int32_t seg_req, burn_req;
     int cus;
+    bool own_stream = true;
+    bool overlap_on = true;
 };
 
 LaunchPlan plan_launch(const Grid& g, const int32_t* ax0, const RunShape& r);
diff --git a/distributed-backtesting-exploration_amd/engine.py b/distributed-backtesting-exploration_amd/engine.py
--- a/distributed-backtesting-exploration_amd/engine.py
+++ b/distributed-backtesting-exploration_amd/engine.py
@@ -221,6 +221,7 @@
                           C.c_void_p], C.c_int32),
     "bt_gram_of": (3, [C.c_void_p, C.c_int32, C.c_int32, C.c_void_p, C.c_void_p, C.c_void_p], C.c_int32),
     "bt_set_gram_split": (3, [C.c_void_p, C.c_int32], C.c_int32),
+    "bt_set_run_overlap": (3, [C.c_void_p, C.c_int32], C.c_int32),
     "bt_covariance_host": (3, [C.c_int32, C.c_void_p, C.c_void_p, C.c_int64, C.c_int32, C.c_int32, C.c_void_p,
                                C.c_void_p, C.c_void_p], C.c_int32),
 }
@@ -705,6 +706,9 @@
     def set_segments(self, segments: int, burn_tiles: int = 0) -> None:
         _check(lib().bt_set_segments(self._h, segments, burn_tiles))
 
+    def set_run_overlap(self, on) -> None:
+        _check(sym("bt_set_run_overlap")(self._h, 1 if on else 0))
+
     def last_segments(self, with_refixed: bool = False):
         n = C.c_int64(0)
         g = _check(lib().bt_last_segments(self._h, C.byref(n)))
diff --git a/include/bt.h b/include/bt.h
--- a/include/bt.h
+++ b/include/bt.h
@@ -101,6 +101,8 @@
 int32_t bt_num_params(const bt_engine* e);
 int32_t bt_set_segments(bt_engine* e, int32_t segments, int32_t burn_tiles);
 int32_t bt_last_segments(bt_engine* e, int64_t* refixed_blocks);
+
+int32_t bt_set_run_overlap(bt_engine* e, int32_t on);
 
 typedef struct bt_batch_profile {
     int64_t n_jobs, n_failed;
```

Result: faster. 5123 billion bar-evals/s (median of 6 runs) (+7.7%).
